# guomc9/CudaRayTracing

Measured on AMD Instinct MI355X. Metric: Mrays/sec, higher is better.
Workload: dtype f32

## Files before the change

### cudaraytracing_amd/_capi.py

```python
import ctypes as C
import os

import numpy as np

from . import build as _build

CRT_OK = 0
ERR_INVALID_ARG, ERR_NO_DEVICE, ERR_HIP = -1, -2, -3
TRAVERSAL_EXACT = 0
TRAVERSAL_REFERENCE = 1
TRAVERSAL_FAST = 2
FLAG_STATS = 1
FLAG_TILED_OUTPUT = 2
FLAG_FORCE_EXACT = 4
FLAG_TRACE_ALL = 8
FLAG_BOUNDED_RADIANCE = 16
FLAG_VARIANCE = 32
GATHER_AUTO, GATHER_RCCL, GATHER_COPY = 0, 1, 2
INTERSECT_RAW_DIRECTIONS, INTERSECT_FORCE_EXACT, INTERSECT_VISIBILITY = 0x100, 0x200, 0x400
TILE = 8


class CrtError(RuntimeError):
    def __init__(self, status, where, detail):
# ... 60 lines not shown
    def as_dict(self):
        d = {n: getattr(self, n) for n, _ in self._fields_}
        d["fallback_reason"] = d["fallback_reason"].decode("utf-8", "replace")
        return d


class BvhBuildInfo(C.Structure):
    _fields_ = [("n_triangles", C.c_uint32), ("n_nodes", C.c_uint32), ("levels", C.c_uint32), ("host_ranges", C.c_uint32),
                ("host_triangles", C.c_uint32), ("host_sorts", C.c_uint32), ("host_sort_elements", C.c_uint64), ("device_ms", C.c_float), ("total_ms", C.c_float), ("host_build_ms", C.c_float)]

    def as_dict(self):
        return {n: getattr(self, n) for n, _ in self._fields_}


class AccelInfo(C.Structure):
    _fields_ = [("n_leaves", C.c_uint32), ("n_nodes2", C.c_uint32), ("n_nodes4", C.c_uint32), ("depth2", C.c_uint32), ("depth4", C.c_uint32),
                ("sah_on_device", C.c_uint32), ("index_splits", C.c_uint32), ("sah_ms", C.c_float), ("sah_device_ms", C.c_float), ("runtime_init_ms", C.c_float), ("layout_caps", C.c_uint32)]

    def as_dict(self):
        return {n: getattr(self, n) for n, _ in self._fields_}


class TreeScalars(C.Structure):
    _fields_ = [("root_fast", C.c_int32), ("root_exact", C.c_int32), ("root3_fast", C.c_int32), ("root3_exact", C.c_int32), ("root4", C.c_int32),
                ("root4i", C.c_int32), ("n_mixed4i", C.c_uint32), ("empty4_off", C.c_uint32), ("empty4i_off", C.c_uint32), ("coord_max", C.c_float),
                ("stack_cap", C.c_uint32), ("node4i_f4", C.c_uint32)]

    def as_dict(self):
        return {n: getattr(self, n) for n, _ in self._fields_}


class AovBuffers(C.Structure):
    _fields_ = [("albedo", C.c_void_p), ("normal", C.c_void_p), ("depth", C.c_void_p), ("coverage", C.c_void_p), ("tri", C.c_void_p),
                ("material", C.c_void_p)]


class AovInfo(C.Structure):
    _fields_ = [("rays", C.c_uint64), ("chunks", C.c_uint32), ("total_ms", C.c_float)]

    def as_dict(self):
        return {n: getattr(self, n) for n, _ in self._fields_}


class DenoiseParams(C.Structure):
    _fields_ = [("width", C.c_uint32), ("height", C.c_uint32), ("iterations", C.c_uint32), ("sigma_color", C.c_float),
                ("sigma_normal", C.c_float), ("sigma_albedo", C.c_float), ("sigma_depth", C.c_float)]


class DenoiseInputs(C.Structure):
    _fields_ = [("color", C.c_void_p), ("albedo", C.c_void_p), ("normal", C.c_void_p), ("depth", C.c_void_p)]


class DenoiseVarInputs(C.Structure):
    _fields_ = [("color", C.c_void_p), ("variance", C.c_void_p), ("albedo", C.c_void_p), ("normal", C.c_void_p), ("depth", C.c_void_p)]


class DenoiseInfo(C.Structure):
    _fields_ = [("total_ms", C.c_float), ("passes", C.c_uint32)]

    def as_dict(self):
        return {n: getattr(self, n) for n, _ in self._fields_}


AOV_BUFFERS = {"albedo": (3, np.float32), "normal": (3, np.float32), "depth": (1, np.float32), "coverage": (1, np.float32),
               "tri": (1, np.int32), "material": (1, np.int32)}


class Task(C.Structure):
    _fields_ = [("n_objs", C.c_uint32), ("obj_path", (C.c_char * 512) * 8), ("mtl_dir", (C.c_char * 512) * 8),
                ("lookat", C.c_float * 3), ("up", C.c_float * 3), ("eye_pos", C.c_float * 3), ("fov_y", C.c_float),
                ("width", C.c_uint32), ("height", C.c_uint32), ("bvh_thresh_n", C.c_uint32),
                ("light_sample_n", C.c_uint32), ("spp", C.c_uint32), ("p_rr", C.c_float)]


NODE_DTYPE = np.dtype([("lc", "<i4"), ("rc", "<i4"), ("n", "<u4"), ("it", "<i4"), ("aa", "<f4", 3), ("bb", "<f4", 3)])
TRI_DTYPE = np.dtype([("v1", "<f4", 3), ("v2", "<f4", 3), ("v3", "<f4", 3), ("normal", "<f4", 3), ("area", "<f4"),
                      ("area_of_obj", "<f4"), ("material", "<i4")])
MAT_DTYPE = np.dtype([("kd", "<f4", 3), ("ke", "<f4", 3), ("ns", "<f4"), ("mode", "<i4"), ("has_emit", "<i4")])
LIGHT_DTYPE = np.dtype([("first_tri", "<u4"), ("count", "<u4")])

ABI_VERSION = 5

EXPORTS = ["crt_strerror", "crt_last_error", "crt_abi_version", "crt_device_count", "crt_scene_create",
           "crt_scene_accel_info", "crt_scene_destroy", "crt_task_obj", "crt_shard_slots", "crt_render", "crt_render_device", "crt_render_range", "crt_render_range_device", "crt_last_launch_ms", "crt_radiance_storage", "crt_preview", "crt_preview_device", "crt_variance", "crt_variance_device", "crt_render_aov", "crt_render_aov_device", "crt_denoise_defaults", "crt_denoise_scratch_bytes", "crt_denoise", "crt_denoise_device", "crt_denoise_var_defaults", "crt_denoise_var", "crt_denoise_var_device", "crt_multi_create", "crt_multi_destroy",
           "crt_multi_render", "crt_multi_frame_device", "crt_intersect",
           "crt_device_math", "crt_device_philox", "crt_device_rcp_check", "crt_scene_export", "crt_host_scene_create", "crt_host_scene_destroy",
           "crt_host_scene_add_obj", "crt_host_scene_set_bvh", "crt_host_scene_set_bvh_device", "crt_host_scene_desc", "crt_host_scene_num_objects",
           "crt_host_scene_object", "crt_inverse_view", "crt_task_load", "crt_image_load", "crt_write_png", "crt_write_pfm"]

_lib = None


def lib_path():
    return _build.LIB


def lib():
    global _lib
    if _lib is not None:
        return _lib
    path = os.environ.get("CRT_LIB_PATH") or _build.build_lib()
    L = C.CDLL(path)
    L.crt_abi_version.restype = C.c_int
    if L.crt_abi_version() != ABI_VERSION:
        raise RuntimeError("%s speaks ABI version %d, these bindings version %d (include/crt.h: CRT_ABI_VERSION)" % (path, L.crt_abi_version(), ABI_VERSION))
    L.crt_strerror.restype = C.c_char_p
    L.crt_strerror.argtypes = [C.c_int]
    L.crt_last_error.restype = C.c_char_p
    L.crt_device_count.argtypes = [C.POINTER(C.c_int)]
    L.crt_scene_create.argtypes = [C.POINTER(SceneDesc), C.c_int, C.POINTER(C.c_void_p)]
    L.crt_scene_accel_info.argtypes = [C.c_void_p, C.POINTER(AccelInfo)]
    L.crt_scene_destroy.argtypes = [C.c_void_p]
    L.crt_shard_slots.argtypes = [C.c_uint32, C.c_uint32, C.c_uint32, C.c_uint32, C.POINTER(C.c_uint64)]
    L.crt_render.argtypes = [C.c_void_p, C.POINTER(Camera), C.POINTER(Params), C.c_void_p, C.c_void_p, C.POINTER(Stats)]
    L.crt_render_device.argtypes = [C.c_void_p, C.POINTER(Camera), C.POINTER(Params), C.c_void_p, C.c_void_p,
                                    C.c_void_p, C.POINTER(Stats)]
    L.crt_render_range.argtypes = [C.c_void_p, C.POINTER(Camera), C.POINTER(Params), C.c_uint32, C.c_uint32, C.c_void_p, C.c_void_p,
                                   C.POINTER(Stats)]
    L.crt_render_range_device.argtypes = [C.c_void_p, C.POINTER(Camera), C.POINTER(Params), C.c_uint32, C.c_uint32, C.c_void_p,
                                          C.c_void_p, C.c_void_p, C.POINTER(Stats)]
    L.crt_last_launch_ms.argtypes = [C.c_void_p, C.POINTER(C.c_float), C.POINTER(C.c_uint32)]
    L.crt_radiance_storage.argtypes = [C.c_void_p, C.POINTER(C.c_uint64), C.POINTER(C.c_uint32)]
    L.crt_preview.argtypes = [C.c_void_p, C.c_void_p, C.c_void_p, C.POINTER(C.c_uint32)]
    L.crt_preview_device.argtypes = [C.c_void_p, C.c_void_p, C.c_void_p, C.c_void_p, C.POINTER(C.c_uint32)]
    L.crt_variance.argtypes = [C.c_void_p, C.c_void_p, C.POINTER(C.c_uint32)]
    L.crt_variance_device.argtypes = [C.c_void_p, C.c_void_p, C.c_void_p, C.POINTER(C.c_uint32)]
    L.crt_render_aov.argtypes = [C.c_void_p, C.POINTER(Camera), C.POINTER(Params), C.POINTER(AovBuffers), C.POINTER(AovInfo)]
    L.crt_render_aov_device.argtypes = [C.c_void_p, C.POINTER(Camera), C.POINTER(Params), C.POINTER(AovBuffers), C.c_void_p,
                                        C.POINTER(AovInfo)]
    L.crt_denoise_defaults.argtypes = [C.POINTER(DenoiseParams)]
    L.crt_denoise_scratch_bytes.argtypes = [C.c_uint32, C.c_uint32, C.POINTER(C.c_uint64)]
    L.crt_denoise.argtypes = [C.c_int, C.POINTER(DenoiseParams), C.POINTER(DenoiseInputs), C.c_void_p, C.c_void_p, C.POINTER(DenoiseInfo)]
    L.crt_denoise_device.argtypes = [C.c_int, C.POINTER(DenoiseParams), C.POINTER(DenoiseInputs), C.c_void_p, C.c_void_p, C.c_void_p, C.c_uint64,
                                     C.c_void_p, C.POINTER(DenoiseInfo)]
    L.crt_denoise_var_defaults.argtypes = [C.POINTER(DenoiseParams)]
    L.crt_denoise_var.argtypes = [C.c_int, C.POINTER(DenoiseParams), C.POINTER(DenoiseVarInputs), C.c_void_p, C.c_void_p, C.c_void_p,
                                  C.POINTER(DenoiseInfo)]
    L.crt_denoise_var_device.argtypes = [C.c_int, C.POINTER(DenoiseParams), C.POINTER(DenoiseVarInputs), C.c_void_p, C.c_void_p, C.c_void_p,
                                         C.c_void_p, C.c_uint64, C.c_void_p, C.POINTER(DenoiseInfo)]
    L.crt_multi_create.argtypes = [C.POINTER(SceneDesc), C.POINTER(C.c_int), C.c_uint32, C.c_uint32, C.POINTER(C.c_void_p)]
    L.crt_multi_destroy.argtypes = [C.c_void_p]
    L.crt_multi_render.argtypes = [C.c_void_p, C.POINTER(Camera), C.POINTER(Params), C.c_void_p, C.c_void_p, C.POINTER(Stats),
                                   C.POINTER(MultiInfo)]
    L.crt_multi_frame_device.argtypes = [C.c_void_p, C.POINTER(C.c_void_p), C.POINTER(C.c_void_p), C.POINTER(C.c_int)]
    L.crt_intersect.argtypes = [C.c_void_p, C.c_uint32, C.c_void_p, C.c_void_p, C.c_uint32, C.c_void_p, C.c_void_p]
    L.crt_device_math.argtypes = [C.c_int, C.c_char_p, C.c_uint32, C.c_void_p, C.c_void_p, C.c_void_p]
    L.crt_device_philox.argtypes = [C.c_int, C.c_uint32, C.c_void_p, C.c_void_p, C.c_void_p]
    L.crt_device_rcp_check.argtypes = [C.c_int, C.POINTER(C.c_uint64), C.POINTER(C.c_uint64)]
    L.crt_scene_export.argtypes = [C.c_void_p, C.c_char_p, C.c_void_p, C.c_size_t, C.POINTER(C.c_size_t)]
    L.crt_host_scene_create.argtypes = [C.c_uint32, C.c_uint32, C.POINTER(C.c_void_p)]
    L.crt_host_scene_destroy.argtypes = [C.c_void_p]
    L.crt_host_scene_add_obj.argtypes = [C.c_void_p, C.c_char_p, C.c_char_p]
    L.crt_host_scene_set_bvh.argtypes = [C.c_void_p, C.c_uint32]
    L.crt_host_scene_set_bvh_device.argtypes = [C.c_void_p, C.c_uint32, C.c_int, C.POINTER(BvhBuildInfo)]
    L.crt_host_scene_desc.argtypes = [C.c_void_p, C.POINTER(SceneDesc)]
    L.crt_host_scene_num_objects.argtypes = [C.c_void_p, C.POINTER(C.c_uint32)]
    L.crt_host_scene_object.argtypes = [C.c_void_p, C.c_uint32, C.POINTER(C.c_float), C.POINTER(C.c_int32),
                                        C.POINTER(C.c_uint32)]
    L.crt_inverse_view.argtypes = [C.c_void_p, C.c_void_p, C.c_void_p, C.c_void_p]
    L.crt_task_load.argtypes = [C.c_char_p, C.POINTER(Task)]
    L.crt_task_obj.argtypes = [C.c_char_p, C.c_uint32, C.c_char_p, C.c_char_p, C.c_uint32]
    L.crt_image_load.argtypes = [C.c_char_p, C.POINTER(C.c_int32), C.POINTER(C.c_int32), C.POINTER(C.c_int32), C.c_void_p, C.c_uint64]
    L.crt_write_png.argtypes = [C.c_char_p, C.c_uint32, C.c_uint32, C.c_void_p]
    L.crt_write_pfm.argtypes = [C.c_char_p, C.c_uint32, C.c_uint32, C.c_uint32, C.c_void_p]
    _lib = L
    return L


def _strerror(status):
    try:
        return lib().crt_strerror(status).decode()
    except Exception:
        return "status"


def check(status, where):
    if status != CRT_OK:
        raise CrtError(status, where, lib().crt_last_error().decode())


def ptr(a):
    return a.ctypes.data_as(C.c_void_p) if a is not None else None
```

### cudaraytracing_amd/api.py

```python
import ctypes as C
import math
import os

import numpy as np

from . import _capi as capi


def get_inverse_view_matrix(eye_pos, lookat, up):
    e = np.asarray(eye_pos, dtype=np.float32)
    l = np.asarray(lookat, dtype=np.float32)
    u = np.asarray(up, dtype=np.float32)
    out = np.zeros(9, dtype=np.float32)
    capi.check(capi.lib().crt_inverse_view(capi.ptr(e), capi.ptr(l), capi.ptr(u), capi.ptr(out)), "crt_inverse_view")
    return out


def fov_to_radians(fov_y_deg):
    return np.float32(np.float32(np.float32(fov_y_deg) * np.float32(math.pi)) / np.float32(180))


class Task:

    def __init__(self, config_path, base_dir=None):
# ... 152 lines not shown
        h = self._handle("export_trees")
        L = capi.lib()
        out = {}
        for name, dt in self.EXPORT_ARRAYS.items():
            n = C.c_size_t()
            capi.check(L.crt_scene_export(h, name.encode(), None, 0, C.byref(n)), "crt_scene_export")
            a = np.zeros(n.value // np.dtype(dt).itemsize, dtype=dt)
            if n.value:
                capi.check(L.crt_scene_export(h, name.encode(), capi.ptr(a), a.nbytes, C.byref(n)), "crt_scene_export")
            out[name] = a.reshape(-1, 4) if dt is np.float32 else a
        s = capi.TreeScalars()
        n = C.c_size_t()
        capi.check(L.crt_scene_export(h, b"scalars", C.byref(s), C.sizeof(s), C.byref(n)), "crt_scene_export")
        assert n.value == C.sizeof(s)
        out.update(s.as_dict())
        return out

    def set_spp(self, spp):
        self.spp = int(spp)

    def set_P_RR(self, p):
        self.P_RR = np.float32(p)

    def set_light_sample_n(self, n):
        self.light_sample_n = int(n)

    def _cam(self, eye_pos, inv_view_mat, fovY):
        cam = capi.Camera()
        cam.eye[:] = [float(v) for v in np.asarray(eye_pos, dtype=np.float32)]
        cam.inv_view[:] = [float(v) for v in np.asarray(inv_view_mat, dtype=np.float32).reshape(9)]
        cam.fov_y = float(np.float32(fovY))
        return cam

    def _params(self, rank=0, world=1, flags=0, width=None, height=None):
        return capi.Params(width or self.scene.width, height or self.scene.height, self.spp, float(self.P_RR),
                           self.light_sample_n, self.seed, rank, world, self.traversal, flags)

    def run_view(self, eye_pos, inv_view_mat, fovY, stats=False, want_mean=True, width=None, height=None, want_variance=False):
        if not self._h:
            raise RuntimeError("Render.run_view after free()")
        cam = self._cam(eye_pos, inv_view_mat, fovY)
        prm = self._params(flags=(capi.FLAG_STATS if stats else 0) | (capi.FLAG_VARIANCE if want_variance else 0) | self.extra_flags,
                           width=width, height=height)
        w, h = prm.width, prm.height
        rgb = np.zeros((h, w, 3), dtype=np.uint8)
        mean = np.zeros((h, w, 3), dtype=np.float32) if want_mean else None
        st = capi.Stats()
        capi.check(capi.lib().crt_render(self._h, C.byref(cam), C.byref(prm), capi.ptr(rgb), capi.ptr(mean),
                                         C.byref(st)), "crt_render")
        self.frame_buffer, self.mean_buffer, self.stats = rgb, mean, st.as_dict()
        self.variance_buffer = self.variance(width=w, height=h)[0] if want_variance else None
        return rgb

    def variance(self, width=None, height=None):
        h_ = self._handle("variance")
        w, h = width or self.scene.width, height or self.scene.height
        var = np.zeros((h, w, 3), dtype=np.float32)
        done = C.c_uint32(0)
        capi.check(capi.lib().crt_variance(h_, capi.ptr(var), C.byref(done)), "crt_variance")
        return var, int(done.value)

    def run_view_range(self, eye_pos, inv_view_mat, fovY, sample_begin, sample_count, want_mean=True, width=None, height=None,
                       want_variance=False):
        if not self._h:
            raise RuntimeError("Render.run_view_range after free()")
        cam = self._cam(eye_pos, inv_view_mat, fovY)
        prm = self._params(flags=(capi.FLAG_VARIANCE if want_variance else 0) | self.extra_flags, width=width, height=height)
        w, h = prm.width, prm.height
        last = sample_begin + sample_count == self.spp
        rgb = np.zeros((h, w, 3), dtype=np.uint8) if last else None
        mean = np.zeros((h, w, 3), dtype=np.float32) if (last and want_mean) else None
        st = capi.Stats()
        capi.check(capi.lib().crt_render_range(self._h, C.byref(cam), C.byref(prm), int(sample_begin), int(sample_count),
                                               capi.ptr(rgb) if last else None, capi.ptr(mean), C.byref(st)), "crt_render_range")
        self.stats = st.as_dict()
        if last:
            self.frame_buffer, self.mean_buffer = rgb, mean
        return rgb

    def last_launch_ms(self):
        ms, n = C.c_float(), C.c_uint32()
        capi.check(capi.lib().crt_last_launch_ms(self._handle("last_launch_ms"), C.byref(ms), C.byref(n)), "crt_last_launch_ms")
        return float(ms.value), int(n.value)

    def radiance_storage(self):
        b, r = C.c_uint64(), C.c_uint32()
        capi.check(capi.lib().crt_radiance_storage(self._handle("radiance_storage"), C.byref(b), C.byref(r)), "crt_radiance_storage")
        return int(b.value), int(r.value)

    def preview(self, want_mean=False, width=None, height=None):
        if not self._h:
            raise RuntimeError("Render.preview after free()")
        w, h = width or self.scene.width, height or self.scene.height
        rgb = np.zeros((h, w, 3), dtype=np.uint8)
        mean = np.zeros((h, w, 3), dtype=np.float32) if want_mean else None
        done = C.c_uint32(0)
        capi.check(capi.lib().crt_preview(self._h, capi.ptr(rgb), capi.ptr(mean), C.byref(done)), "crt_preview")
        return rgb, mean, int(done.value)

    def run_view_device(self, eye_pos, inv_view_mat, fovY, d_rgb_ptr, d_mean_ptr=None, stream=None, rank=0, world=1,
                        tiled=False, want_stats=True, width=None, height=None):
        self._handle("run_view_device")
        cam = self._cam(eye_pos, inv_view_mat, fovY)
        flags = (capi.FLAG_TILED_OUTPUT if (tiled or world > 1) else 0) | self.extra_flags
        prm = self._params(rank=rank, world=world, flags=flags, width=width, height=height)
        st = capi.Stats()
        capi.check(capi.lib().crt_render_device(self._h, C.byref(cam), C.byref(prm), C.c_void_p(d_rgb_ptr),
                                                C.c_void_p(d_mean_ptr) if d_mean_ptr else None,
                                                C.c_void_p(stream) if stream else None,
                                                C.byref(st) if want_stats else None), "crt_render_device")
        if want_stats:
            self.stats = st.as_dict()
        return self.stats

    def run_view_aov(self, eye_pos, inv_view_mat, fovY, want=tuple(capi.AOV_BUFFERS), width=None, height=None):
        h_ = self._handle("run_view_aov")
        cam = self._cam(eye_pos, inv_view_mat, fovY)
        prm = self._params(flags=self.extra_flags, width=width, height=height)
        w, h = prm.width, prm.height
        out, bufs = {}, capi.AovBuffers()
        for name in want:
            ch, dt = capi.AOV_BUFFERS[name]
            out[name] = np.zeros((h, w, 3) if ch == 3 else (h, w), dtype=dt)
            setattr(bufs, name, out[name].ctypes.data)
        info = capi.AovInfo()
        capi.check(capi.lib().crt_render_aov(h_, C.byref(cam), C.byref(prm), C.byref(bufs), C.byref(info)), "crt_render_aov")
        self.aov_info = info.as_dict()
        return out

    def run_view_aov_device(self, eye_pos, inv_view_mat, fovY, ptrs, stream=None, rank=0, world=1, tiled=False, want_info=True,
                            width=None, height=None):
        h_ = self._handle("run_view_aov_device")
        cam = self._cam(eye_pos, inv_view_mat, fovY)
        flags = (capi.FLAG_TILED_OUTPUT if (tiled or world > 1) else 0) | self.extra_flags
        prm = self._params(rank=rank, world=world, flags=flags, width=width, height=height)
        bufs = capi.AovBuffers()
        for name, p in ptrs.items():
            if name not in capi.AOV_BUFFERS:
                raise ValueError("unknown AOV buffer %r" % name)
            setattr(bufs, name, int(p) if p else None)
        info = capi.AovInfo()
        capi.check(capi.lib().crt_render_aov_device(h_, C.byref(cam), C.byref(prm), C.byref(bufs), C.c_void_p(stream) if stream else None,
                                                    C.byref(info) if want_info else None), "crt_render_aov_device")
        if want_info:
            self.aov_info = info.as_dict()
        return self.aov_info if want_info else None

    def run_view_denoised(self, eye_pos, inv_view_mat, fovY, iterations=None, sigma_color=None, sigma_normal=None, sigma_albedo=None,
                          sigma_depth=None, width=None, height=None, variance_guided=False):
        self._handle("run_view_denoised")
        self.run_view(eye_pos, inv_view_mat, fovY, width=width, height=height, want_variance=variance_guided)
        self.aov_buffers = self.run_view_aov(eye_pos, inv_view_mat, fovY, want=("albedo", "normal", "depth"), width=width, height=height)
        if variance_guided:
            rgb, mean, self.denoise_info = denoise_var(self.mean_buffer, self.variance_buffer, iterations=iterations, sigma_color=sigma_color,
                                                       sigma_normal=sigma_normal, sigma_albedo=sigma_albedo, sigma_depth=sigma_depth,
                                                       device=self.device, return_info=True, **self.aov_buffers)
            return rgb, mean
        rgb, mean, self.denoise_info = denoise(self.mean_buffer, iterations=iterations, sigma_color=sigma_color, sigma_normal=sigma_normal,
                                               sigma_albedo=sigma_albedo, sigma_depth=sigma_depth, device=self.device, return_info=True,
                                               **self.aov_buffers)
        return rgb, mean

    def intersect(self, origins, dirs, traversal=None):
        self._handle("intersect")
        o = np.ascontiguousarray(origins, dtype=np.float32)
        d = np.ascontiguousarray(dirs, dtype=np.float32)
# ... 293 lines not shown
```

### cudaraytracing_amd/csrc/crt_mega3.h

```cpp
#ifndef CRT_MEGA3_H
#define CRT_MEGA3_H
#include "crt_path.h"

namespace crtk {

struct MParams {
    LParams P;
    DevScene sc;
    unsigned long long* counters;
    int2* spill;
    uint32_t spill_stride;
    int32_t stack_cap;
    int32_t logic_min, leaf_min;
};

#define POOL_LV 4

#define PH3_INNER 0
#define PH3_LEAF 1
#define PH3_LA 2
#define PH3_LB 3
#define PH3_LC 4
#define PH3_N 5
#define PH3_WAIT 5
#define PH3_NONE 7
#define RF_ANYHIT 0x1000000u
#define RF_SHADOW 0x2000000u
#define RF_LAST 0x4000000u
#define RF_PROBE 0x8000000u
#define RR_ROUTE_SHIFT 25
#define RR_ROUTE_MASK 0x6000000u
#define RR_ROUTE_LC_BIT 0x4000000u
#define RF_EXACT 0x10000000u
#define RF_HASHIT 0x20000000u
#define RF_SKIP 0x40000000u
#define RF_QUERY 0x80000000u
#define POOL3_P 164
#define POOL3_QCAP ((POOL3_P + 3) & ~3)
static_assert(POOL3_P <= 256, "ray ids of a pool must fit a byte (ring entries are uint8_t)");
static_assert(POOL3_QCAP >= POOL3_P, "a ring must hold every ray of the pool");
#define CRT_MEGA3_MAX_STACK 255
#define CRT_MEGA3_MAX_LEAF 65535

typedef float v2f __attribute__((ext_vector_type(2)));

#define CRT_WAVES 4
template <bool R16_>
struct Pool3LdsT {
    static constexpr bool R16 = R16_;
    static constexpr bool DEC = false;
    static constexpr int P = POOL3_P, QCAP = POOL3_QCAP;
    static constexpr int LV = R16_ ? 2 * POOL_LV : POOL_LV;
    typedef typename std::conditional<R16_, short, int>::type stk_t;
    float4 A[POOL3_P];
    float4 B[POOL3_P];
    int node[POOL3_P];
    stk_t stk[LV][POOL3_P];
    uint32_t D[POOL3_P];
    uint8_t ring[PH3_N + 1][POOL3_QCAP];
    uint32_t waitq;
    __device__ __forceinline__ uint8_t* rq(const int p) { return ring[p]; }
};
typedef Pool3LdsT<false> Pool3Lds;
static_assert(sizeof(Pool3LdsT<true>) == sizeof(Pool3Lds), "16-bit stack entries: twice the levels in the same bytes");
static_assert(sizeof(Pool3Lds) * 4 * CRT_WAVES <= 160 * 1024, "the pool does not fit CRT_WAVES waves per SIMD into 160 KiB of LDS");

#ifndef LEAFQ_CAP
#define LEAFQ_CAP 256
#endif
static_assert((LEAFQ_CAP & (LEAFQ_CAP - 1)) == 0 && LEAFQ_CAP >= 128, "leaf queue: a power of two, room for half a batch of inner steps");
#define RD_PEND_SHIFT 8
#define RD_PEND_MASK 0x3ff00u
#define RD_FIN 0x8000000u
#define LEAF_REC_MAX 0x7fffffu
template <bool R16_, bool RING_>
struct Pool4LdsT {
    static constexpr bool R16 = R16_;
    static constexpr bool DEC = true;
    static constexpr int P = RING_ ? 148 : 152;
    static constexpr int QCAP = (P + 3) & ~3;
    static constexpr int LV = R16_ ? 6 : 3;
    typedef typename std::conditional<R16_, short, int>::type stk_t;
    float4 A[P];
    float4 B[P];
    unsigned long long best[P];
    stk_t stk[LV][P];
    uint32_t D[P];
    uint32_t leafq[LEAFQ_CAP + 1];
    uint8_t ring[(RING_ ? 5 : 4)][QCAP];
    uint32_t waitq;
    __device__ __forceinline__ uint8_t* rq(const int p) { return ring[p == PH3_INNER ? 0 : p - 1]; }
};
static_assert(sizeof(Pool4LdsT<true, false>) * 4 * CRT_WAVES <= 160 * 1024 && sizeof(Pool4LdsT<true, true>) * 4 * CRT_WAVES <= 160 * 1024 &&
              sizeof(Pool4LdsT<false, false>) * 4 * CRT_WAVES <= 160 * 1024 && sizeof(Pool4LdsT<false, true>) * 4 * CRT_WAVES <= 160 * 1024,
              "the DEC pool does not fit CRT_WAVES waves per SIMD into 160 KiB of LDS");
static_assert(Pool4LdsT<true, false>::P <= 256, "ray ids of a pool must fit a byte");

struct MParams3 {
    MParams M;
    int* spill;
    uint32_t force_exact;
    int32_t dbg_loads, dbg_valu;
};

static_assert(offsetof(MParams3, dbg_loads) == 748 && offsetof(MParams3, dbg_valu) == 752, "tools/bbprof/instrument.py reads the counter buffer's address from these two kernel-argument dwords");


typedef void (*Mega3Kernel)(const MParams3);
Mega3Kernel mega3_kernel(int mode, bool stats, bool all, bool query, bool r16, bool ring = false, bool dec = false, bool impl = false);
uint32_t mega3_pool_p(bool dec, bool ring);
int mega3_lds_levels(bool dec, bool r16);
bool bbprof_launch(Mega3Kernel kern, MParams3 M3, uint32_t blocks, hipStream_t st);
void launch_order_items(bool ring, uint32_t blocks, hipStream_t st, const LParams& P, uint32_t* list, unsigned int* cnt);

}
#endif
```

### cudaraytracing_amd/csrc/crt_mega3.hip

```cpp
#include "crt_internal.h"

#include <cstdio>
#include <cstdlib>
#include <cstring>
#include <vector>

namespace crtk {

struct NewRay {
    F3 o, d;
    float tl;
    uint32_t kind, flags;
};

__device__ __forceinline__ float fmin3(float a, float b, float c) { return __builtin_fminf(__builtin_fminf(a, b), c); }
__device__ __forceinline__ float fmax3(float a, float b, float c) { return __builtin_fmaxf(__builtin_fmaxf(a, b), c); }
__device__ __forceinline__ v2f v2(float a, float b) { v2f r; r.x = a; r.y = b; return r; }
__device__ __forceinline__ v2f v2s(float a) { v2f r; r.x = a; r.y = a; return r; }

__device__ __forceinline__ int smax(const int a, const int b)
{
    int r;
    asm("s_max_i32 %0, %1, %2" : "=s"(r) : "s"(a), "s"(b) : "scc");
    return r;
// ... 39 lines not shown
    uint32_t flags = (nr.flags & ~(RF_SKIP | RF_SHADOW | RF_LAST | RF_PROBE)) | route_bits(nr.flags);
    const float max_o = __builtin_elementwise_maximum(__builtin_elementwise_maximum(absf(nr.o.x), absf(nr.o.y)), absf(nr.o.z));
    const float max_inv = __builtin_elementwise_maximum(__builtin_elementwise_maximum(absf(inv.x), absf(inv.y)), absf(inv.z));
    const bool finite = ((sc.coord_max + max_o) * max_inv <= 0x1p126f) & finite3(nr.d.x, nr.d.y, nr.d.z);
    if (MODE == 1 || !finite || force_exact) flags |= RF_EXACT;
    const int ref = (MODE != 1 && finite && !force_exact) ? (IMPL ? sc.root4i : sc.root4) : sc.root3_exact;
    bool answered = false;
    float T = FLT_MAX;
    if (MODE != 1 && nr.kind == RAY_SHADOW) {
        flags |= RF_ANYHIT;
        T = nr.tl;
        answered = !(nr.tl == nr.tl) || nr.tl == -pinf() || (nr.flags & RF_SKIP) != 0;
    }
    if constexpr (LDS::DEC) {
        static_assert(!LDS::DEC || MODE == 2, "decoupled leaves: CRT_TRAVERSAL_EXACT");
        if (ref < 0) flags |= RF_EXACT;
        S.A[id] = make_float4(nr.o.x, nr.o.y, nr.o.z, (flags & RF_ANYHIT) ? T : pinf());
        S.B[id] = make_float4(nr.d.x, nr.d.y, nr.d.z, __int_as_float(ref));
        S.best[id] = (unsigned long long)0x7f7fffffu << 32;
        S.D[id] = flags;
        enters_exact = false;
        if (answered) return route_done<QUERY>(flags);
        enters_exact = (flags & RF_EXACT) != 0;
        return PH3_INNER;
    } else {
    S.A[id] = make_float4(nr.o.x, nr.o.y, nr.o.z, T);
    S.B[id] = make_float4(nr.d.x, nr.d.y, nr.d.z, __int_as_float(-1));
    S.node[id] = ref;
    S.D[id] = flags;
    enters_exact = false;
    if (answered) return route_done<QUERY>(flags);
    enters_exact = MODE != 1 && (flags & RF_EXACT) != 0;
    return ref >= 0 ? PH3_INNER : PH3_LEAF;
    }
}

template <class LDS>
__device__ __forceinline__ void ray_result(LDS& S, const uint32_t id, float4& qa, float4& qb)
{
    qa = S.A[id]; qb = S.B[id];
    if constexpr (LDS::DEC) {
        const unsigned long long b = S.best[id];
        qa.w = __uint_as_float((uint32_t)(b >> 32));
        qb.w = __uint_as_float(~(uint32_t)b);
    }
}
template <bool QUERY>
__device__ __forceinline__ uint32_t route_complete(const uint32_t rec_flags, const bool has_hit)
{
    if (QUERY) return PH3_LC;
    const uint32_t r = (rec_flags >> RR_ROUTE_SHIFT) & 3u;
    return (has_hit ? (r & 1u) : r) + (uint32_t)PH3_LA;
}

template <int MODE>
__device__ __forceinline__ bool shadow_blocked(float tl, float T, int tri)
{
    if (MODE != 1) return tri >= 0 || tl - FLT_MAX > CRT_EPSILON;
    return tl - T > CRT_EPSILON;
}

__device__ __forceinline__ F3 finish_path_m3(const LParams& P, const Tables<false>& tb, const uint32_t slot, const int deepest, const bool emissive, const F3 ke,
                                            const bool have_ld, const F3 ld)
{
    const Pool& pl = P.pool;
    F3 L = f3(0.0f, 0.0f, 0.0f);
    if (deepest < 0) return L;
    const float inv_pdf_sphere = (float)(2.0f * 3.14159265358979323846);
    if (emissive) {
        L = deepest == 0 ? add3(f3(0.0f, 0.0f, 0.0f), ke) : f3(0.0f, 0.0f, 0.0f);
    } else if (have_ld) {
        L = add3(f3(0.0f, 0.0f, 0.0f), ld);
    } else {
        const float4 a = gld_rec(&pl.rec_a[(size_t)deepest * pl.n + slot]);
        L = add3(f3(0.0f, 0.0f, 0.0f), f3(a.x, a.y, a.z));
    }
    for (int v = deepest - 1; v >= 0; v -= CRT_FINISH_PF) {
        float4 a[CRT_FINISH_PF], fm[CRT_FINISH_PF];
        float cs[CRT_FINISH_PF];
#pragma unroll
        for (int j = 0; j < CRT_FINISH_PF; j++) {
            const int vj = v - j > 0 ? v - j : 0;
            a[j] = gld_rec(&pl.rec_a[(size_t)vj * pl.n + slot]);
            cs[j] = __uint_as_float(gld((const uint32_t*)&pl.rec_b[(size_t)vj * pl.n + slot].w));
        }
#pragma unroll
        for (int j = 0; j < CRT_FINISH_PF; j++) fm[j] = mat_row(tb, TNM_MAT(__float_as_uint(a[j].w)), 0);
#pragma unroll
        for (int j = 0; j < CRT_FINISH_PF; j++) {
            if (v - j >= 0) {
                F3 ind = mul3(L, f3(fm[j].x, fm[j].y, fm[j].z));
                ind = scale3(ind, cs[j]);
                ind = scale3(ind, inv_pdf_sphere);
                ind = div3(ind, P.p_rr);
                L = add3(ind, f3(a[j].x, a[j].y, a[j].z));
            }
        }
    }
    return L;
}

__device__ __forceinline__ bool shadow_blocked_bit(const bool tl_inf, const int tri) { return tri >= 0 || tl_inf; }
#define ST_TL_INF (1u << 12)

template <int MODE, bool RING = false>
__device__ __forceinline__ uint32_t logic_A(const LParams& P, const Tables<false>& tb, const uint32_t g, const float4 qa, const float4 qb, NewRay& nr,
                                            PathCounters& cnt, const bool trace_all)
{
    const DevScene& sc = P.sc;
    const Pool& pl = P.pool;
    constexpr bool TRI_CC = MODE != 1;
    const float4 la = gld(&pl.la[g]);
    const uint4 idv = load_path_id<RING, !TRI_CC>(P, g);
    const float4 cc = gld(&pl.cc[g]);
    const uint32_t st = __float_as_uint(la.w);
    const uint32_t stage = (st >> 8) & 15u;
    const uint32_t vtri_old = TRI_CC ? ((st & 0xfffu) == ((uint32_t)ST_HIT << 8) ? 0u : __float_as_uint(cc.w)) : idv.w;
    const float4 vn = gld(&sc.tri_nm[vtri_old]);
    const float res_t = qa.w;
    const int res_tri = __float_as_int(qb.w);
    const float4 gq_hit = gld(&sc.tri_nm[res_tri >= 0 ? res_tri : 0]);
    const uint32_t mat_old = min(TNM_MAT(__float_as_uint(vn.w)), P.n_mats - 1u);
    const uint32_t mat_cur = stage == ST_HIT ? TNM_MAT(__float_as_uint(gq_hit.w)) : mat_old;
    uint32_t tnm_cur = stage == ST_HIT ? __float_as_uint(gq_hit.w) : __float_as_uint(vn.w);
    float4 m0_cur = mat_row(tb, mat_cur, 0);
    const uint32_t n_nee = (uint32_t)(sc.n_lights * P.lsn);
    const uint32_t q_next = stage == ST_SHADOW ? (st >> 16) + 1 : 0u;
    uint4 lg_next = make_uint4(0u, 1u, 0u, 0u);
    if (n_nee > 0) {
        if (sc.n_lights == 1) {
            const crt_u4v_ l0_ = *(const __attribute__((address_space(4))) crt_u4v_*)tb.lights;
            lg_next = make_uint4(l0_.x, l0_.y, l0_.z, l0_.w);
        } else lg_next = gld(&tb.lights[fast_div(q_next < n_nee ? q_next : 0u, P.lsn_div.m, P.lsn_div.sh)]);
    }
    Lane s;
    s.depth = st & 255u; s.q = st >> 16; s.stage = stage;
    s.Ld = f3(la.x, la.y, la.z);
    s.nrm = f3(vn.x, vn.y, vn.z); s.mat = TNM_MAT(__float_as_uint(vn.w));
    s.pixel_index = idv.x; s.k = idv.y; s.item = idv.z;
    s.ro = f3(qa.x, qa.y, qa.z); s.tl = 0.0f;
    s.rd = f3(qb.x, qb.y, qb.z);
    s.pos = s.ro; s.vtri = vtri_old; s.c = f3(0.0f, 0.0f, 0.0f); s.kind = RAY_NONE;
    bool do_enter = false;
    if (stage == ST_SHADOW) {
        const bool blocked = TRI_CC ? shadow_blocked_bit((st & ST_TL_INF) != 0u, res_tri) : shadow_blocked<MODE>(cc.w, res_t, res_tri);
        if (!blocked) s.Ld = add3(s.Ld, f3(cc.x, cc.y, cc.z));
        s.q++;
    } else if (stage == ST_HIT) {
        const F3 pos = add3(s.ro, scalel3(res_t, s.rd));
        do_enter = true;
        if (s.depth > 0) {
            const size_t pr = (size_t)(s.depth - 1) * pl.n + g;
            const F3 pn = s.nrm;
            float cos_prev = dot3(unit3(sub3(pos, s.ro)), pn);
            cos_prev = cos_prev > 0.0f ? cos_prev : 0.0f;
            gst_rec(&pl.rec_b[pr].w, cos_prev);
            if (TNM_SPECULAR(__float_as_uint(vn.w))) {
                const float ns = mat_row(tb, s.mat, 0).w;
                const float4 pb = gld_rec(&pl.rec_b[pr]);
                const float delta_coeff = (float)((double)(det_expf(25 / ns) - 1) / (2.71828182845904523536 - 1));
                const F3 in = unit3(f3(pb.x, pb.y, pb.z));
                const F3 out = sub3(in, scale3(pn, 2.f * dot3(in, pn)));
                const float d_theta = (float)((double)(delta_coeff * 30) * 3.14159265358979323846 / 180);
                const float d_phi = (float)((double)(delta_coeff * 120) * 3.14159265358979323846 / 180);
                const U4 rp = rng_draw(P.seed, s.pixel_index, s.k, s.depth - 1, RNG_PROBE, 0);
                const F3 refd = unit3(sample_lobe(out, d_theta, d_phi, rng_uniform(rp.x), rng_uniform(rp.y)));
                gst_rec(&pl.rec_b[(size_t)s.depth * pl.n + g], make_float4(s.rd.x, s.rd.y, s.rd.z, 0.0f));
                gst(&pl.vx[g], make_float4(pos.x, pos.y, pos.z, __int_as_float(res_tri)));
                gst(&pl.la[g], make_float4(s.Ld.x, s.Ld.y, s.Ld.z, __uint_as_float(s.depth | ((uint32_t)ST_PROBE << 8) | (s.q << 16))));
                nr.o = s.ro; nr.d = unit3(refd);  nr.tl = 0.0f; nr.kind = RAY_CLOSEST; nr.flags = RF_PROBE;
                return PH3_NONE;
            }
        }
        s.pos = pos; s.vtri = (uint32_t)res_tri;
    } else {
        const float4 vx = gld(&pl.vx[g]);
        s.pos = f3(vx.x, vx.y, vx.z); s.vtri = __float_as_uint(vx.w);
        if (res_tri >= 0) {
            const int hmat = gld(&sc.tri_mat[res_tri]);
            const float4 h1 = mat_row(tb, hmat, 1);
            if (__float_as_uint(h1.w) & 1u) {
                const float4 h2 = mat_row(tb, hmat, 2);
                const size_t pr = (size_t)(s.depth - 1) * pl.n + g;
                const F3 pn = s.nrm;
                const float4 pm0 = mat_row(tb, s.mat, 0), pm1 = mat_row(tb, s.mat, 1);
                const float log_shininess = det_log10f(pm0.w);
                const float shininess_coeff = (float)((double)log_shininess * 0.5 + 1);
                const float ip = (float)(2.0f * 3.14159265358979323846) / 8.f;
                const F3 hp = add3(s.ro, scalel3(res_t, s.rd));
                float ct = dot3(unit3(sub3(hp, s.ro)), pn);
                ct = ct > 0.0f ? ct : 0.0f;
                const F3 kekd = mul3(f3(h2.x, h2.y, h2.z), f3(pm1.x, pm1.y, pm1.z));
                const F3 temp = scale3(scale3(scalel3(shininess_coeff, kekd), ct), ip);
                float4 a = gld_rec(&pl.rec_a[pr]);
                a.x = a.x + temp.x; a.y = a.y + temp.y; a.z = a.z + temp.z;
                gst_rec(&pl.rec_a[pr], a);
            }
        }
        const float4 pb = gld_rec(&pl.rec_b[(size_t)s.depth * pl.n + g]);
        s.rd = f3(pb.x, pb.y, pb.z);
        do_enter = true;
    }
    if (do_enter) {
        float4 gq = gq_hit;
        if (stage == ST_PROBE) {
            gq = gld(&sc.tri_nm[s.vtri]);
            m0_cur = mat_row(tb, TNM_MAT(__float_as_uint(gq.w)), 0); tnm_cur = __float_as_uint(gq.w);
        }
        s.nrm = f3(gq.x, gq.y, gq.z);
        s.mat = TNM_MAT(__float_as_uint(gq.w));
        if (TNM_SPECULAR(tnm_cur)) gst_rec(&pl.rec_b[(size_t)s.depth * pl.n + g], make_float4(s.rd.x, s.rd.y, s.rd.z, 0.0f));
        if (!TRI_CC) store_path_tri(P, g, s.vtri);
        if (TNM_EMITTER(tnm_cur)) {
            gst(&pl.la[g], make_float4(TRI_CC ? __uint_as_float(s.vtri) : 0.0f, 0.0f, 0.0f, __uint_as_float(s.depth | ((uint32_t)ST_FIN << 8) | (1u << 16))));
            return PH3_LC;
        }
        s.Ld = f3(0.0f, 0.0f, 0.0f);
        s.q = 0;
        if (n_nee == 0) {
            gst(&pl.la[g], make_float4(0.0f, 0.0f, 0.0f, __uint_as_float(s.depth | ((uint32_t)ST_NEED << 8))));
            if (TRI_CC) gst(&pl.cc[g].w, __uint_as_float(s.vtri));
            nr.o = s.pos;
            return PH3_LB;
        }
    }
    constexpr int LA_LOOP_MIN = 16;
    const float4 m0 = m0_cur;
    bool skip;
    for (bool first = true;; first = false) {
        if (first) setup_shadow_lg(P, s, f3(m0.x, m0.y, m0.z), lg_next);
        else setup_shadow(P, tb, s, f3(m0.x, m0.y, m0.z));
        skip = MODE != 1 && !trace_all && (s.c.x == 0.0f && s.c.y == 0.0f && s.c.z == 0.0f);
        if (!skip) break;
        cnt.untraced++;
        if (__popcll(__builtin_amdgcn_ballot_w64(true)) < LA_LOOP_MIN) break;
        cnt.rays++; cnt.shadow++;
        s.q++;
        if (s.q == n_nee) {
            gst(&pl.la[g], make_float4(s.Ld.x, s.Ld.y, s.Ld.z, __uint_as_float(s.depth | ((uint32_t)ST_NEED << 8))));
            if (TRI_CC) gst(&pl.cc[g].w, __uint_as_float(s.vtri));
            nr.o = s.pos;
            return PH3_LB;
        }
    }
    gst(&pl.la[g], make_float4(s.Ld.x, s.Ld.y, s.Ld.z, __uint_as_float(s.depth | ((uint32_t)ST_SHADOW << 8) | (s.q << 16) | ((TRI_CC && s.tl == pinf()) ? ST_TL_INF : 0u))));
    gst(&pl.cc[g], make_float4(s.c.x, s.c.y, s.c.z, TRI_CC ? __uint_as_float(s.vtri) : s.tl));
    nr.o = s.ro; nr.d = s.rd; nr.tl = s.tl; nr.kind = RAY_SHADOW;
    nr.flags = RF_SHADOW | (s.q + 1 == n_nee ? RF_LAST : 0u) | (skip ? RF_SKIP : 0u);
    return PH3_NONE;
}

template <int MODE, bool RING = false>
__device__ __forceinline__ uint32_t logic_B(const LParams& P, const uint32_t g, const float4 qa, const float4 qb, NewRay& nr)
{
    const Pool& pl = P.pool;
    constexpr bool TRI_CC = MODE != 1;
    const float4 la = gld(&pl.la[g]);
    const uint4 idv = load_path_id<RING, !TRI_CC>(P, g);
    const float4 cc = gld(&pl.cc[g]);
    const uint32_t st = __float_as_uint(la.w);
    const uint32_t stage = (st >> 8) & 15u;
    uint32_t depth = st & 255u;
    F3 Ld = f3(la.x, la.y, la.z);
    if (stage == ST_SHADOW) {
        const bool blocked = TRI_CC ? shadow_blocked_bit((st & ST_TL_INF) != 0u, __float_as_int(qb.w)) : shadow_blocked<MODE>(cc.w, qa.w, __float_as_int(qb.w));
        if (!blocked) Ld = add3(Ld, f3(cc.x, cc.y, cc.z));
    }
    bool stop = depth == CRT_BOUNCE_STACK_SIZE - 1;
    U4 rb;
    rb.x = rb.y = rb.z = rb.w = 0;
    if (!stop) {
        rb = rng_draw(P.seed, idv.x, idv.y, depth, RNG_BOUNCE, 0);
        stop = rng_uniform(rb.x) > P.p_rr;
    }
    if (stop) {
        gst(&pl.la[g], make_float4(Ld.x, Ld.y, Ld.z, __uint_as_float(depth | ((uint32_t)ST_FIN << 8))));
        return PH3_LC;
    }
    const float4 vn = gld(&P.sc.tri_nm[TRI_CC ? __float_as_uint(cc.w) : idv.w]);
    const float4 vx = qa;
    gst_rec(&pl.rec_a[(size_t)depth * pl.n + g], make_float4(Ld.x, Ld.y, Ld.z, vn.w));
    const F3 ndir = unit3(sample_hemisphere(f3(vn.x, vn.y, vn.z), rng_uniform(rb.y), rng_uniform(rb.z)));
    depth++;
    gst(&pl.la[g], make_float4(Ld.x, Ld.y, Ld.z, __uint_as_float(depth | ((uint32_t)ST_HIT << 8))));
    nr.o = f3(vx.x, vx.y, vx.z); nr.d = unit3(ndir);  nr.tl = 0.0f; nr.kind = RAY_CLOSEST; nr.flags = 0;
    return PH3_NONE;
}

enum { LC_DEAD = 0, LC_RAY = 1, LC_WAIT = 2 };
template <int MODE, bool RING>
__device__ __forceinline__ int logic_C(const LParams& P, const Tables<false>& tb, const uint32_t g, PathCounters& cnt, NewRay& nr, uint32_t& fin_key)
{
    constexpr bool TRI_CC = MODE != 1;
    const Pool& pl = P.pool;
    const float4 la = gld(&pl.la[g]);
    const uint4 idv = load_path_id<RING, !TRI_CC>(P, g);
    const uint32_t st = __float_as_uint(la.w);
    const uint32_t stage = (st >> 8) & 15u;
    const uint32_t depth = st & 255u;
    constexpr bool ring = RING;
    const bool waiting = ring && stage == ST_WAIT;
    const uint32_t home_ = RING ? blockIdx.x & (P.ring_shards - 1u) : blockIdx.x & (ITEM_SHARDS - 1);
    const uint32_t lo_ = home_ * P.items_per_shard, hi_ = min(lo_ + P.items_per_shard, P.n_items);
    const unsigned long long gmask_ = __ballot(!waiting);
    const int lane_ = threadIdx.x & 63;
    const uint32_t grank_ = (uint32_t)__popcll(gmask_ & ((1ull << lane_) - 1ull));
    unsigned int pre_base_ = 0;
    const bool pre_ok_ = lo_ < P.n_items && gmask_ != 0ull;
    if (pre_ok_ && lane_ == __ffsll((long long)gmask_) - 1) pre_base_ = __hip_atomic_fetch_add((CRT_GAS unsigned int*)(P.item_next + home_ * ITEM_STRIDE), (unsigned int)__popcll(gmask_), __ATOMIC_RELAXED, __HIP_MEMORY_SCOPE_AGENT);
    uint32_t home_word_ = 0;
    if (RING) home_word_ = ring_load(P.ring_state + home_ * ITEM_STRIDE);
    if (stage != ST_NEW && !waiting) {
        int deepest = (int)depth;
        bool emissive = false;
        F3 ke = f3(0.0f, 0.0f, 0.0f);
        if (stage == ST_HIT) deepest = (int)depth - 1;
        else if ((st >> 16) & 1u) {
            emissive = true;
            const float4 m2 = mat_row(tb, TNM_MAT(__float_as_uint(gld(&P.sc.tri_nm[TRI_CC ? __float_as_uint(la.x) : idv.w]).w)), 2);
            ke = f3(m2.x, m2.y, m2.z);
        }
        const F3 L = finish_path_m3(P, tb, g, deepest, emissive, ke, stage == ST_FIN && !emissive, f3(la.x, la.y, la.z));
        if (ring) {
            const uint32_t sh = fast_div(idv.z, P.items_per_shard_div.m, P.items_per_shard_div.sh), c = idv.z - sh * P.items_per_shard;
            const uint32_t s = fast_div(c, P.spsh_div.m, P.spsh_div.sh), rs = s & P.ring_mask;
            float4* Lr = P.L + (size_t)rs * P.ring_stride + (size_t)sh * P.spsh + (c - s * P.spsh);
            ring_store16(Lr, L.x, L.y, L.z);
            fin_key = (sh << 16) | rs;
        } else {
            typedef float f4v_ __attribute__((ext_vector_type(4)));
            f4v_ Lv_; Lv_.x = L.x; Lv_.y = L.y; Lv_.z = L.z; Lv_.w = 0.0f;
            __builtin_nontemporal_store(Lv_, (CRT_GAS f4v_*)&P.L[idv.z]);
        }
    }
    bool first_ = pre_ok_ && !waiting;
    for (;;) {
        uint32_t item = ITEM_NONE;
        if (waiting) item = idv.z;
        else {
            if (first_) {
                const unsigned long long idx_ = (unsigned long long)lo_ + (unsigned int)__builtin_amdgcn_readfirstlane((int)pre_base_) + grank_;
                if (idx_ < hi_) item = (uint32_t)idx_;
                first_ = false;
            }
            if (item == ITEM_NONE) item = RING ? grab_item_ring(P.item_next, P.items_per_shard, P.ring_shards, home_)
                                               : grab_item(nullptr, P.item_next, P.items_per_shard, P.n_items, blockIdx.x & (ITEM_SHARDS - 1));
            if (item == ITEM_NONE) return LC_DEAD;
            if (P.item_list) {
                const uint32_t sh_ = fast_div(item, P.items_per_shard_div.m, P.items_per_shard_div.sh);
                const uint32_t slo_ = sh_ * P.items_per_shard, shi_ = min(slo_ + P.items_per_shard, P.n_items);
                const uint32_t wlo_ = shi_ - min(P.order_window, shi_ - slo_);
                if (item >= wlo_) item = __hip_atomic_load((CRT_GAS const unsigned int*)&P.item_list[sh_ * P.order_window + (item - wlo_)], __ATOMIC_RELAXED, __HIP_MEMORY_SCOPE_AGENT);
            }
        }
        bool valid; uint32_t pi, pj, pixel_index, k;
        decode_item<RING>(P, item, pixel_index, k, valid, pi, pj);
        if (!valid) continue;
        if (ring && !ring_gate_open(P, item, home_, home_word_)) {
            if (!waiting) {
                store_path_id<!TRI_CC>(P, g, item);
                gst(&pl.la[g], make_float4(0.0f, 0.0f, 0.0f, __uint_as_float((uint32_t)ST_WAIT << 8)));
            }
            return LC_WAIT;
        }
        cnt.paths++;
        if (!waiting) store_path_id<!TRI_CC>(P, g, item);
        const F3 wd = camera_dir(P, pixel_index, k, pi, pj);
        gst(&pl.la[g], make_float4(0.0f, 0.0f, 0.0f, __uint_as_float((uint32_t)ST_HIT << 8)));
        nr.o = f3(P.eye[0], P.eye[1], P.eye[2]); nr.d = unit3(wd);  nr.tl = 0.0f; nr.kind = RAY_CLOSEST; nr.flags = 0;
        return LC_RAY;
    }
}

__device__ __forceinline__ bool query_C(const LParams& P, const uint32_t g, const float4 qa, const float4 qb, NewRay& nr)
{
    const Pool& pl = P.pool;
    const float4 la = gld(&pl.la[g]);
    const uint4 idv = load_path_id(P, g);
    if (((__float_as_uint(la.w) >> 8) & 15u) != ST_NEW) gst(&P.L[idv.z], make_float4(qa.w, qb.w, 0.0f, 0.0f));
    const uint32_t item = grab_item(nullptr, P.item_next, P.items_per_shard, P.n_items, blockIdx.x & (ITEM_SHARDS - 1));
    if (item == ITEM_NONE) return false;
    store_path_id(P, g, item);
    gst(&pl.la[g], make_float4(0.0f, 0.0f, 0.0f, __uint_as_float((uint32_t)ST_HIT << 8)));
    const float4 o = gld(&P.q_o[item]), d = gld(&P.q_d[item]);
    nr.o = f3(o.x, o.y, o.z); nr.d = f3(d.x, d.y, d.z); nr.tl = o.w; nr.kind = __float_as_uint(d.w); nr.flags = RF_QUERY;
    return true;
}

__device__ __forceinline__ void slab_pair(const float4 n0, const float4 n1, const float4 n2, const F3 o, const F3 inv, const F3 d, const bool exact,
                                          bool& hl, bool& hr, float& tl, float& tr)
{
    const v2f tx0 = (v2(n0.x, n0.y) - v2s(o.x)) * v2s(inv.x), ty0 = (v2(n0.z, n0.w) - v2s(o.y)) * v2s(inv.y), tz0 = (v2(n1.x, n1.y) - v2s(o.z)) * v2s(inv.z);
    const v2f tx1 = (v2(n1.z, n1.w) - v2s(o.x)) * v2s(inv.x), ty1 = (v2(n2.x, n2.y) - v2s(o.y)) * v2s(inv.y), tz1 = (v2(n2.z, n2.w) - v2s(o.z)) * v2s(inv.z);
    float el, er, xl, xr;
    if (!exact) {
        el = fmax3(__builtin_fminf(tx0.x, tx1.x), __builtin_fminf(ty0.x, ty1.x), __builtin_fminf(tz0.x, tz1.x));
        er = fmax3(__builtin_fminf(tx0.y, tx1.y), __builtin_fminf(ty0.y, ty1.y), __builtin_fminf(tz0.y, tz1.y));
        xl = fmin3(__builtin_fmaxf(tx0.x, tx1.x), __builtin_fmaxf(ty0.x, ty1.x), __builtin_fmaxf(tz0.x, tz1.x));
        xr = fmin3(__builtin_fmaxf(tx0.y, tx1.y), __builtin_fmaxf(ty0.y, ty1.y), __builtin_fmaxf(tz0.y, tz1.y));
    } else {
        const bool nx = d.x < 0, ny = d.y < 0, nz = d.z < 0;
        el = maxf_ref(maxf_ref(nx ? tx1.x : tx0.x, ny ? ty1.x : ty0.x), nz ? tz1.x : tz0.x);
        er = maxf_ref(maxf_ref(nx ? tx1.y : tx0.y, ny ? ty1.y : ty0.y), nz ? tz1.y : tz0.y);
        xl = minf_ref(minf_ref(nx ? tx0.x : tx1.x, ny ? ty0.x : ty1.x), nz ? tz0.x : tz1.x);
        xr = minf_ref(minf_ref(nx ? tx0.y : tx1.y, ny ? ty0.y : ty1.y), nz ? tz0.y : tz1.y);
    }
    hl = (el <= xl + CRT_EPSILON) & (xl >= 0);
    hr = (er <= xr + CRT_EPSILON) & (xr >= 0);
    tl = el; tr = er;
}

__device__ __forceinline__ void slab_pair_pruned(const float4 n0, const float4 n1, const float4 n2, const F3 o, const F3 inv, const float bound,
                                                 float& tl, float& tr)
{
    const v2f tx0 = (v2(n0.x, n0.y) - v2s(o.x)) * v2s(inv.x), ty0 = (v2(n0.z, n0.w) - v2s(o.y)) * v2s(inv.y), tz0 = (v2(n1.x, n1.y) - v2s(o.z)) * v2s(inv.z);
    const v2f tx1 = (v2(n1.z, n1.w) - v2s(o.x)) * v2s(inv.x), ty1 = (v2(n2.x, n2.y) - v2s(o.y)) * v2s(inv.y), tz1 = (v2(n2.z, n2.w) - v2s(o.z)) * v2s(inv.z);
    const float el = fmax3(__builtin_fminf(tx0.x, tx1.x), __builtin_fminf(ty0.x, ty1.x), __builtin_fminf(tz0.x, tz1.x));
    const float er = fmax3(__builtin_fminf(tx0.y, tx1.y), __builtin_fminf(ty0.y, ty1.y), __builtin_fminf(tz0.y, tz1.y));
    const float xl = fmin3(__builtin_fmaxf(tx0.x, tx1.x), __builtin_fmaxf(ty0.x, ty1.x), __builtin_fmaxf(tz0.x, tz1.x));
    const float xr = fmin3(__builtin_fmaxf(tx0.y, tx1.y), __builtin_fmaxf(ty0.y, ty1.y), __builtin_fmaxf(tz0.y, tz1.y));
    const float inf = pinf();
    tl = ((el <= __builtin_fminf(xl + CRT_EPSILON, bound)) & (xl >= 0)) ? el : inf;
    tr = ((er <= __builtin_fminf(xr + CRT_EPSILON, bound)) & (xr >= 0)) ? er : inf;
}

template <bool PRUNE = true>
__device__ __forceinline__ void slab_quad_pruned(const float4 nx, const float4 fx, const float4 ny, const float4 fy, const float4 nz, const float4 fz,
                                                 const F3 o, const F3 inv, const float bound, float& t0, float& t1, float& t2, float& t3)
{
    const v2f nxa = (v2(nx.x, nx.y) - v2s(o.x)) * v2s(inv.x), nxb = (v2(nx.z, nx.w) - v2s(o.x)) * v2s(inv.x);
    const v2f nya = (v2(ny.x, ny.y) - v2s(o.y)) * v2s(inv.y), nyb = (v2(ny.z, ny.w) - v2s(o.y)) * v2s(inv.y);
    const v2f nza = (v2(nz.x, nz.y) - v2s(o.z)) * v2s(inv.z), nzb = (v2(nz.z, nz.w) - v2s(o.z)) * v2s(inv.z);
    const v2f fxa = (v2(fx.x, fx.y) - v2s(o.x)) * v2s(inv.x), fxb = (v2(fx.z, fx.w) - v2s(o.x)) * v2s(inv.x);
    const v2f fya = (v2(fy.x, fy.y) - v2s(o.y)) * v2s(inv.y), fyb = (v2(fy.z, fy.w) - v2s(o.y)) * v2s(inv.y);
    const v2f fza = (v2(fz.x, fz.y) - v2s(o.z)) * v2s(inv.z), fzb = (v2(fz.z, fz.w) - v2s(o.z)) * v2s(inv.z);
    const float e0 = fmax3(nxa.x, nya.x, nza.x), e1 = fmax3(nxa.y, nya.y, nza.y), e2 = fmax3(nxb.x, nyb.x, nzb.x), e3 = fmax3(nxb.y, nyb.y, nzb.y);
    const float x0 = fmin3(fxa.x, fya.x, fza.x), x1 = fmin3(fxa.y, fya.y, fza.y), x2 = fmin3(fxb.x, fyb.x, fzb.x), x3 = fmin3(fxb.y, fyb.y, fzb.y);
    const float inf = pinf();
    if (PRUNE) {
        t0 = ((e0 <= __builtin_fminf(x0 + CRT_EPSILON, bound)) & (x0 >= 0)) ? e0 : inf;
        t1 = ((e1 <= __builtin_fminf(x1 + CRT_EPSILON, bound)) & (x1 >= 0)) ? e1 : inf;
        t2 = ((e2 <= __builtin_fminf(x2 + CRT_EPSILON, bound)) & (x2 >= 0)) ? e2 : inf;
        t3 = ((e3 <= __builtin_fminf(x3 + CRT_EPSILON, bound)) & (x3 >= 0)) ? e3 : inf;
    } else {
        t0 = ((e0 <= x0 + CRT_EPSILON) & (x0 >= 0)) ? e0 : inf;
        t1 = ((e1 <= x1 + CRT_EPSILON) & (x1 >= 0)) ? e1 : inf;
        t2 = ((e2 <= x2 + CRT_EPSILON) & (x2 >= 0)) ? e2 : inf;
        t3 = ((e3 <= x3 + CRT_EPSILON) & (x3 >= 0)) ? e3 : inf;
    }
}

// ... 316 lines not shown
}

template <int MODE, bool STATS, class LDS>
__device__ __forceinline__ bool inner2_step(const DevScene& sc, LDS& S, const MParams3& M, const uint32_t id, const uint32_t g, const F3 o, const F3 inv,
                                            const F3 d, const float bound, int& ref, int& sp, TravCounters& tc, uint32_t& max_sp)
{
    const float4* nd = sc.nodes3 + (size_t)ref * 4;
    const float4 n0 = nd[0], n1 = nd[1], n2 = nd[2];
    const float2 n3 = *(const float2*)(nd + 3);
    if (STATS) tc.inner++;
    bool hl, hr;
    float tl, tr;
    slab_pair(n0, n1, n2, o, inv, d, true, hl, hr, tl, tr);
    const int lref = __float_as_int(n3.x), rref = __float_as_int(n3.y);
    bool left_first;
    if (MODE == 1) {
        left_first = false;
    } else {
        hl = hl && !(tl > bound);
        hr = hr && !(tr > bound);
        left_first = tl <= tr;
    }
    const bool both = hl && hr, any = hl || hr;
    const int near_ref = both ? (left_first ? lref : rref) : (hl ? lref : rref);
    const int lv = lds_levels<LDS>(true);
    if (both) {
        stack_push(S, M, id, g, sp, left_first ? rref : lref, lv);
        if (STATS && (uint32_t)sp > max_sp) max_sp = (uint32_t)sp;
    }
    if (any) { ref = near_ref; return false; }
    return stack_pop(S, M, id, g, sp, ref, lv);
}

#define CRT_SORT4(mode) ((mode) != 2)
template <int MODE, bool STATS, bool ALL = false, bool QUERY = false, bool R16 = false, bool RING = false, bool DEC = false, bool IMPL = false>
__global__ __launch_bounds__(64) __attribute__((amdgpu_waves_per_eu(CRT_WAVES, CRT_WAVES))) void k_mega3(const MParams3 M3)
{
    static_assert(!IMPL || (DEC && R16), "the tree without its rows of refs: decoupled leaves, 16-bit stack entries");
    static_assert(!(RING && (QUERY || STATS)), "the commit ring is a render without counters");
    static_assert(!(R16 && MODE == 1), "CRT_TRAVERSAL_REFERENCE walks the 2-wide trees: 32-bit stack entries");
    static_assert(!DEC || MODE == 2, "decoupled leaves: CRT_TRAVERSAL_EXACT");
    typedef typename std::conditional<DEC, Pool4LdsT<R16, RING>, Pool3LdsT<R16>>::type LDS3;
    __shared__ LDS3 S;
    constexpr int QCAP = LDS3::QCAP;
    const MParams& M = M3.M;
    const LParams& P = M.P;
    const DevScene& sc = P.sc;
    const Pool& pl = P.pool;
    const int lane = threadIdx.x;
    const uint32_t base = blockIdx.x * (uint32_t)LDS3::P;
    Tables<false> tb;
    tb.mats = sc.mats; tb.lights = sc.lights;

    PathCounters cnt;
    cnt = PathCounters{};
    TravCounters tc;
    tc.inner = tc.leaf = tc.tests = tc.hits = 0;
    uint32_t max_sp = 0;
    int n_exact = 0;

    int qn[PH3_N];
#pragma unroll
    for (int p = 0; p < PH3_N; p++) qn[p] = 0;
    uint32_t dg_b[5] = {0, 0, 0, 0, 0}, dg_l[5] = {0, 0, 0, 0, 0};
    uint32_t dg_sp[6] = {0, 0, 0, 0, 0, 0};
    uint32_t dg_ov[2] = {0, 0};
    uint32_t lq_h = 0, lq_t = 0;
    constexpr bool commit_ring = RING;
#ifdef CRT_STAMPS
    unsigned long long st_acc[6] = {0, 0, 0, 0, 0, 0};
    uint32_t st_n[6] = {0, 0, 0, 0, 0, 0};
    unsigned long long st_prev = __builtin_amdgcn_s_memtime();
#define STAMP(k_) { const unsigned long long t_ = __builtin_amdgcn_s_memtime(); st_acc[k_] += t_ - st_prev; st_prev = t_; st_n[k_]++; }
#define STAMP_OTHER() { const unsigned long long t_ = __builtin_amdgcn_s_memtime(); st_acc[3] += t_ - st_prev; st_prev = t_; }
#else
#define STAMP(k_)
#define STAMP_OTHER()
#endif
    if (commit_ring && lane == 0) S.waitq = 0u;
    {
        const int n_valid = __builtin_amdgcn_readfirstlane((int)min((uint32_t)LDS3::P, pl.n > base ? pl.n - base : 0u));
        for (int i = lane; i < n_valid; i += 64) {
            S.rq(PH3_LC)[i] = (uint8_t)i;
            pl.la[base + i] = make_float4(0.0f, 0.0f, 0.0f, __uint_as_float((uint32_t)ST_NEW << 8));
        }
        qn[PH3_LC] = n_valid;
    }

#define PUSH3()                                                                                                            \
    _Pragma("unroll") for (int p = 0; p < PH3_N; p++) {                                                                    \
        const bool mine = nph == (uint32_t)p;                                                                         \
        const unsigned long long m = __ballot(mine);                                                                       \
        if (m) {                                                                                                           \
                  \
            const uint32_t slot = __builtin_amdgcn_mbcnt_hi((uint32_t)(m >> 32), __builtin_amdgcn_mbcnt_lo((uint32_t)m, RQ_PUSH_BASE(p))); \
            if (mine) S.rq(p)[slot] = (uint8_t)id;                                                                             \
            const int add = (int)__popcll(m);                                                                              \
            RQ_PUSH_ADV(p, add)                                                                                            \
        }                                                                                                                  \
    }
#define PUSH_TRAV() { if (on) nph = t_done ? route_done<QUERY>(t_flags) : (t_ref >= 0 ? PH3_INNER : PH3_LEAF); PUSH3() }
#define POP3(p)                                                                                                            \
    const int take = min(64, qn[p]);                                                                                       \
    if (STATS) { dg_b[p]++; dg_l[p] += (uint32_t)take; }                                                                   \
    const bool on = lane < take;                                                                                           \
    const uint32_t id = S.rq(p)[RQ_POP_BASE(p, take) + (uint32_t)lane];                                                        \
    RQ_POP_ADV(p, take)                                                                                                    \
    const uint32_t g = base + id;                                                                                          \
    uint32_t nph = PH3_NONE;

#define LOGIC_PARAMS()                                                                                                     \
    const __attribute__((address_space(4))) char* ka_ = (const __attribute__((address_space(4))) char*)__builtin_amdgcn_kernarg_segment_ptr(); \
    asm volatile("" : "+s"(ka_));                                                                                          \
    union { LParams p; uint32_t w[sizeof(LParams) / 4]; } pu_;                                                             \
    {                                                                                                                      \
        const __attribute__((address_space(4))) uint32_t* src_ =                                                           \
            (const __attribute__((address_space(4))) uint32_t*)(ka_ + offsetof(MParams3, M) + offsetof(MParams, P));       \
        _Pragma("unroll") for (unsigned i_ = 0; i_ < sizeof(LParams) / 4; i_++) pu_.w[i_] = src_[i_];                      \
    }                                                                                                                      \
    const LParams& Pl = pu_.p;                                                                                             \
    Tables<false> tl;                                                                                                      \
    tl.mats = Pl.sc.mats; tl.lights = Pl.sc.lights;

    for (;;) {
      int act;
      for (;;) {
        {
            const int kC = min(qn[PH3_LC], 64) * 8 + PH3_LC, kA = min(qn[PH3_LA], 64) * 8 + PH3_LA, kB = min(qn[PH3_LB], 64) * 8 + PH3_LB;
#define LEAFQ_FIRST 48
            static_assert(LEAFQ_FIRST >= 1 && LEAFQ_FIRST + 64 + 4 <= LEAFQ_CAP, "leaf queue: LEAFQ_FIRST - 1 entries + a reference-arithmetic batch + one lane's four entries must fit LEAFQ_CAP");
            const int nl_ = DEC ? (int)(lq_t - lq_h) : qn[PH3_LEAF];
            const int kL = ((DEC && nl_ >= LEAFQ_FIRST) ? 64 : min(nl_, 64)) * 8 + PH3_LEAF, kI = min(qn[PH3_INNER], 64) * 8 + PH3_INNER;
            const int best = STATS ? max(max(max(kC, kA), max(kB, kL)), kI)
                                   : smax(smax(smax(kC, kA), smax(kB, kL)), kI);
            act = best < 8 ? PH3_NONE : (best & 7);
        }
        if (act > PH3_LEAF) break;
        auto inner_arm = [&](auto may_exact_) __attribute__((always_inline)) {
            constexpr bool MAY_EXACT = decltype(may_exact_)::value;
            if constexpr (!DEC) {
            POP3(PH3_INNER)
            bool t_done = false;
            int t_ref = 0;
            uint32_t t_flags = 0;
            if (on) {
                const float4 qa = S.A[id], qbd = S.B[id];
                const uint32_t qd = S.D[id];
                int ref = S.node[id];
                constexpr bool DIR_ = MODE == 2 && !MAY_EXACT;
                const F3 o = f3(qa.x, qa.y, qa.z), inv = DIR_ ? f3(qbd.x, qbd.y, qbd.z) : inv3_exact(f3(qbd.x, qbd.y, qbd.z));
                int sp = (int)(qd & 0xffu);
                const float bound = (MODE == 0 && (qd & (RF_ANYHIT | RF_HASHIT))) ? prune_bound(qa.w, o, inv) : pinf();
                bool done = false;
                if (MODE == 1) {
                    const float4 qb = S.B[id];
                    done = inner2_step<1, STATS>(sc, S, M3, id, g, o, inv, f3(qb.x, qb.y, qb.z), bound, ref, sp, tc, max_sp);
                } else if (!MAY_EXACT) {
                    done = inner4_step<STATS, CRT_SORT4(MODE), LDS3, DIR_>(sc, S, M3, id, g, o, inv, bound, ref, sp, tc, max_sp);
                } else {
                    const bool ex = (qd & RF_EXACT) != 0;
                    if (!ex) done = inner4_step<STATS, CRT_SORT4(MODE)>(sc, S, M3, id, g, o, inv, bound, ref, sp, tc, max_sp);
                    if (__builtin_amdgcn_ballot_w64(ex)) {
                        if (ex) {
                            const float4 qb = S.B[id];
                            done = inner2_step<0, STATS>(sc, S, M3, id, g, o, inv, f3(qb.x, qb.y, qb.z), bound, ref, sp, tc, max_sp);
                        }
                    }
// ... 560 lines not shown
```

### cudaraytracing_amd/csrc/crt_path.h

```cpp
#ifndef CRT_PATH_H
#define CRT_PATH_H
#include "../../include/crt.h"
#include "crt_accel.h"
#include "crt_device.h"
#include "crt_trace.h"

#include <hip/hip_runtime.h>

#include <cfloat>
#include <cstddef>
#include <cstdint>
#include <type_traits>

namespace crtk {
using namespace crtdev;

enum { C_RAYS = 0, C_SHADOW, C_PROBE, C_INNER, C_LEAF, C_TESTS, C_HITS, C_PATHS, C_ALIVE, C_MAXSP, C_SUMSP, C_CYC_LOGIC, C_CYC_LEAF, C_CYC_INNER, C_CYC_OTHER,
       C_DIAG , C_UNTRACED = C_DIAG + 20, C_COUNT };
#define CNT_SHARDS 256
#define CNT_STRIDE 40
#define ITEM_SHARDS 64
#define ITEM_STRIDE 32

enum { ST_DEAD = 0, ST_NEW = 1, ST_HIT = 2, ST_PROBE = 3, ST_SHADOW = 4, ST_FIN = 5, ST_NEED = 6, ST_WAIT = 7, ST_COUNT_ };
static_assert(ST_COUNT_ <= 16, "a stage is kept in 4 bits");
enum { RAY_NONE = 0, RAY_CLOSEST = 1, RAY_SHADOW = 2 };
#define ITEM_NONE 0xffffffffu

struct Pool {
    float4* ro;
    float4* rd;
    float4* vx;
    float4* la;
    float4* cc;
    float4* vn;
    uint4* id;
    float2* res;
    float4* rec_a;
    float4* rec_b;
    uint32_t n;
};

struct LParams {
    DevScene sc;
    Pool pool;
    float eye[3];
    float inv_view[9];
    float scale, ar;
    uint32_t width, height;
    float p_rr;
    int32_t lsn;
    float inv_lsn_pow2;
    uint32_t pad_;
    uint64_t seed;
    uint32_t rank, world, tiles_x, n_tiles;
    uint32_t nslots;
    uint32_t sample_begin;
    uint32_t n_items;
    uint32_t items_per_shard;
    uint32_t n_mats;
    FastDiv lsn_div, nslots_div, tiles_x_div;
    unsigned int* item_next;
    float4* L;
    unsigned long long* counters;
    const float4* q_o;
    const float4* q_d;
    const uint32_t* item_list;
    uint32_t order_window;
    FastDiv items_per_shard_div;
    uint32_t ring_mask;
    uint32_t spsh;
    FastDiv spsh_div;
    uint32_t ring_shards;
    uint32_t ring_stride;
    uint32_t n_samples;
    uint32_t tail_first;
    float spp_f;
    uint32_t ring_pad_;
    unsigned int* ring_done;
    unsigned int* ring_state;
    float* accum;
};

struct TParams {
    DevScene sc;
    Pool pool;
    unsigned long long* counters;
    unsigned int* slot_next;
    uint32_t slots_per_shard;
    int32_t stack_cap;
    int2* spill;
    uint32_t spill_stride;
    int32_t refill_min, leaf_min;
};

__device__ __forceinline__ bool slot_to_pixel(uint32_t slot, uint32_t rank, uint32_t world, uint32_t n_tiles, uint32_t tiles_x, FastDiv tiles_x_div,
                                              uint32_t width, uint32_t height, uint32_t& i, uint32_t& j)
{
    uint32_t tile = (slot >> 6) * world + rank;
    uint32_t pix = slot & 63u;
    if (tile >= n_tiles) return false;
    uint32_t ty = fast_div(tile, tiles_x_div.m, tiles_x_div.sh), tx = tile - ty * tiles_x;
    i = tx * CRT_TILE + (pix & 7u);
    j = ty * CRT_TILE + (pix >> 3);
    return i < width && j < height;
}

#define CRT_GAS __attribute__((address_space(1)))
typedef float crt_f4v_ __attribute__((ext_vector_type(4)));
typedef uint32_t crt_u4v_ __attribute__((ext_vector_type(4)));
__device__ __forceinline__ float4 gld(const float4* p) { const crt_f4v_ v = *(const CRT_GAS crt_f4v_*)p; return make_float4(v.x, v.y, v.z, v.w); }
__device__ __forceinline__ uint4 gld(const uint4* p) { const crt_u4v_ v = *(const CRT_GAS crt_u4v_*)p; return make_uint4(v.x, v.y, v.z, v.w); }
__device__ __forceinline__ int32_t gld(const int32_t* p) { return *(const CRT_GAS int32_t*)p; }
__device__ __forceinline__ uint32_t gld(const uint32_t* p) { return *(const CRT_GAS uint32_t*)p; }
__device__ __forceinline__ void gst(float4* p, const float4 v) { crt_f4v_ t; t.x = v.x; t.y = v.y; t.z = v.z; t.w = v.w; *(CRT_GAS crt_f4v_*)p = t; }
__device__ __forceinline__ void gst(uint4* p, const uint4 v) { crt_u4v_ t; t.x = v.x; t.y = v.y; t.z = v.z; t.w = v.w; *(CRT_GAS crt_u4v_*)p = t; }
__device__ __forceinline__ void gst(float* p, const float v) { *(CRT_GAS float*)p = v; }
__device__ __forceinline__ float4 gld_rec(const float4* p) { return gld(p); }
__device__ __forceinline__ void gst_rec(float4* p, const float4 v) { gst(p, v); }
__device__ __forceinline__ void gst_rec(float* p, const float v) { gst(p, v); }

__device__ __forceinline__ uint32_t grab_item(const unsigned int* , unsigned int* item_next, uint32_t per, uint32_t n_items,
                                              uint32_t home)
{
    const int lane = threadIdx.x & 63;
    uint32_t item = ITEM_NONE;
    for (uint32_t t = 0; t < ITEM_SHARDS; t++) {
        const uint32_t sh = (home + t) & (ITEM_SHARDS - 1);
        const uint32_t lo = sh * per;
        if (lo >= n_items) continue;
        const uint32_t hi = min(lo + per, n_items);
        unsigned int* cur = item_next + sh * ITEM_STRIDE;
        if (lo + __hip_atomic_load((CRT_GAS unsigned int*)cur, __ATOMIC_RELAXED, __HIP_MEMORY_SCOPE_AGENT) >= hi) continue;
        const unsigned long long mask = __ballot(1);
        const int leader = __ffsll((long long)mask) - 1;
        const uint32_t rank = (uint32_t)__popcll(mask & ((1ull << lane) - 1ull));
// ... 339 lines not shown
```

### cudaraytracing_amd/csrc/crt_render.hip

```cpp
#include "crt_internal.h"

#include <algorithm>
#include <cfloat>
#include <chrono>
#include <cstdio>
#include <cstdlib>
#include <cstring>
#include <limits>
#include <string>
#include <type_traits>
#include <array>
#include <atomic>
#include <vector>

using namespace crtdev;
using namespace crtk;

struct crt_scene {
    int device = 0;
    DevBuf<float4> nodes, tri_geo, mats, ltri, nodes3, leaf_geo, tri_nm, nodes4, nodes4i, leaf_geo_i;
    DevBuf<int32_t> rec_map;
    bool impl_ok = false;
    int depth4 = 1;
    bool ref16_ok = false;
    bool ref16_inner_ok = false;
    bool dec_ok = false;
    uint32_t max_leaf = 0;
    DevBuf<int32_t> tri_mat, leaf_count;
    DevBuf<uint4> lights;
    DevBuf<float4> p_ro, p_rd, p_vx, p_la, p_cc, p_vn, p_rec_a, p_rec_b, L;
    DevBuf<uint4> p_id;
    uint32_t n_mats = 0;
    DevBuf<float2> p_res;
    DevBuf<float> accum;
    DevBuf<float4> aov_acc;
    DevBuf<unsigned long long> counters;
    DevBuf<unsigned int> item_next;
    DevBuf<uint32_t> item_list;
    DevBuf<unsigned int> ring_done, ring_state;
    DevBuf<float4> ring_L;
    std::vector<unsigned int> ring_state_host;
    uint64_t last_radiance_bytes = 0;
    uint32_t last_ring_samples = 0;
    DevBuf<unsigned int> order_cnt;
    DevBuf<unsigned int> slot_next[2];
    DevBuf<int2> spill[2];
    hipStream_t aux_stream = nullptr;
    hipEvent_t ev_fork = nullptr, ev_join = nullptr;
    hipEvent_t ev_k0 = nullptr, ev_k1 = nullptr;
    uint32_t last_launches = 0;
    int n_cus = 0;
    unsigned long long* h_counters = nullptr;
    DevScene dev{};
    int stack_cap = 0;
    uint32_t n_tris = 0;
    crt_accel_info accel{};
    struct { uint32_t samples = 0, spp = 0, width = 0, height = 0, rank = 0, world = 1, tiled = 0; } acc;
    DevBuf<float> accum_q;
    struct { uint32_t samples = 0, spp = 0, width = 0, height = 0, rank = 0, world = 1, tiled = 0; bool valid = false; } var;
    std::vector<hipEvent_t> ev;
    ~crt_scene()
    {
        for (hipEvent_t e : ev) (void)hipEventDestroy(e);
        if (ev_k0) (void)hipEventDestroy(ev_k0);
        if (ev_k1) (void)hipEventDestroy(ev_k1);
        if (ev_fork) (void)hipEventDestroy(ev_fork);
        if (ev_join) (void)hipEventDestroy(ev_join);
        if (aux_stream) (void)hipStreamDestroy(aux_stream);
        if (h_counters) (void)hipHostFree(h_counters);
    }
};

static bool use_ref16(const crt_scene* sc, int mode, bool dec = false)
{
    if (mode == 1 || !(dec ? sc->ref16_inner_ok : sc->ref16_ok)) return false;
    const char* e = std::getenv("CRT_REF16");
    const char* f = std::getenv("CRT_REF32");
    if (f && f[0] == '1') return false;
    return dec || !(e && e[0] == '0');
}

namespace {

int fail(int status, const std::string& msg)
{
    crt_set_last_error_(msg.c_str());
    return status;
}
int fail_hip(const HipFail& f)
{
    return fail(CRT_ERR_HIP, std::string(f.what) + ": " + hipGetErrorString(f.e));
}

float as_float(int32_t v) { float f; std::memcpy(&f, &v, 4); return f; }
int32_t as_int(float f) { int32_t v; std::memcpy(&v, &f, 4); return v; }

struct AccelInfo {
    uint32_t n_leaves = 0, n_nodes2 = 0, on_device = 0, index_splits = 0;
    float sah_ms = 0.0f, sah_device_ms = 0.0f;
};
int convert_bvh(const crt_scene_desc& d, std::vector<float4>& nodes, std::vector<int32_t>& leaf_count, int32_t& root_fast, int32_t& root_exact, AccelInfo* ai = nullptr)
{
    auto is_leaf = [&](int32_t i) { return d.nodes[i].lc < 0 && d.nodes[i].rc < 0; };
    auto leaf_ref = [&](int32_t i) -> int32_t {
        const crt_bvh_node& n = d.nodes[i];
        uint32_t cnt = n.n <= 15 ? n.n : 0;
        if (n.n > 15) leaf_count[n.it] = (int32_t)n.n;
        return (int32_t)~(((uint32_t)n.it << 4) | cnt);
    };
    leaf_count.assign(d.n_tris ? d.n_tris : 1, 0);
    nodes.clear();
    if (is_leaf(d.root)) { root_fast = root_exact = leaf_ref(d.root); return 1; }

    std::vector<crtaccel::Prim> prims;
    for (uint32_t i = 0; i < d.n_nodes; i++) {
        if (!is_leaf((int32_t)i)) continue;
        crtaccel::Prim p;
        for (int a = 0; a < 3; a++) { p.box.lo[a] = d.nodes[i].aa[a]; p.box.hi[a] = d.nodes[i].bb[a]; }
        p.ref = leaf_ref((int32_t)i);
        prims.push_back(p);
    }
    std::vector<crtaccel::Node> acc;
    int32_t acc_root = 0;
    const auto sah_t0 = std::chrono::steady_clock::now();
    int depth_fast = -1;
// ... 63 lines not shown
int validate_desc(const crt_scene_desc* d)
{
    if (!d || !d->nodes || !d->tris || !d->materials || d->n_nodes == 0 || d->n_tris == 0 || d->n_materials == 0)
        return fail(CRT_ERR_INVALID_ARG, "crt_scene_create: empty scene description");
    if (d->root < 0 || (uint32_t)d->root >= d->n_nodes) return fail(CRT_ERR_INVALID_ARG, "crt_scene_create: root index out of range");
    if (d->n_tris >= (1u << 27)) return fail(CRT_ERR_UNSUPPORTED, "crt_scene_create: more than 2^27 triangles");
    if (d->n_lights && (!d->lights || !d->light_tris)) return fail(CRT_ERR_INVALID_ARG, "crt_scene_create: lights without triangles");
    for (uint32_t i = 0; i < d->n_nodes; i++) {
        const crt_bvh_node& n = d->nodes[i];
        bool leaf = n.lc < 0 && n.rc < 0;
        if (leaf) {
            if (n.it < 0 || n.n == 0 || (uint64_t)n.it + n.n > d->n_tris) return fail(CRT_ERR_INVALID_ARG, "crt_scene_create: leaf range outside the triangle array");
        } else {
            if (n.lc < 0 || n.rc < 0 || (uint32_t)n.lc >= i || (uint32_t)n.rc >= i) return fail(CRT_ERR_INVALID_ARG, "crt_scene_create: inner node children must precede it (post-order)");
        }
    }
    {
        std::vector<uint8_t> seen(d->n_nodes, 0), owned(d->n_tris, 0);
        std::vector<int32_t> todo(1, d->root);
        uint32_t visited = 0;
        while (!todo.empty()) {
            const int32_t i = todo.back();
            todo.pop_back();
            if (seen[i]) return fail(CRT_ERR_INVALID_ARG, "crt_scene_create: a node is reachable from the root more than once");
            seen[i] = 1;
            visited++;
            const crt_bvh_node& n = d->nodes[i];
            if (n.lc < 0 && n.rc < 0) {
                for (uint32_t k = 0; k < n.n; k++) {
                    if (owned[(uint32_t)n.it + k]) return fail(CRT_ERR_INVALID_ARG, "crt_scene_create: two leaves share a triangle");
                    owned[(uint32_t)n.it + k] = 1;
                }
            } else { todo.push_back(n.lc); todo.push_back(n.rc); }
        }
        if (visited != d->n_nodes) return fail(CRT_ERR_INVALID_ARG, "crt_scene_create: nodes that the root does not reach");
    }
    if (d->n_materials >= (1u << 30)) return fail(CRT_ERR_INVALID_ARG, "crt_scene_create: more than 2^30 - 1 materials (the triangle rows keep two flag bits beside the index)");
    for (uint32_t i = 0; i < d->n_tris; i++)
        if (d->tris[i].material < 0 || (uint32_t)d->tris[i].material >= d->n_materials) return fail(CRT_ERR_INVALID_ARG, "crt_scene_create: triangle material index out of range");
    for (uint32_t i = 0; i < d->n_light_tris; i++)
        if (d->light_tris[i].material < 0 || (uint32_t)d->light_tris[i].material >= d->n_materials) return fail(CRT_ERR_INVALID_ARG, "crt_scene_create: light triangle material index out of range");
    for (uint32_t i = 0; i < d->n_lights; i++)
        if (d->lights[i].count == 0 || (uint64_t)d->lights[i].first_tri + d->lights[i].count > d->n_light_tris) return fail(CRT_ERR_INVALID_ARG, "crt_scene_create: light range outside the light triangle array");
    return CRT_OK;
}

struct Shard {
    uint32_t tiles_x, tiles_y, n_tiles, local_tiles, nslots;
};
struct RingPlan { uint32_t samples, spsh, shards; };
Shard make_shard(uint32_t w, uint32_t h, uint32_t world)
{
    Shard s;
    s.tiles_x = (w + CRT_TILE - 1) / CRT_TILE;
    s.tiles_y = (h + CRT_TILE - 1) / CRT_TILE;
    s.n_tiles = s.tiles_x * s.tiles_y;
    s.local_tiles = (s.n_tiles + world - 1) / world;
    s.nslots = s.local_tiles * 64u;
    return s;
}

float inv_if_pow2(int32_t n) { return (n > 0 && (n & (n - 1)) == 0) ? 1.0f / (float)n : 0.0f; }

uint32_t env_u32(const char* name, uint32_t dflt)
{
    const char* v = std::getenv(name);
    if (!v || !*v) return dflt;
    long x = std::strtol(v, nullptr, 10);
    return x > 0 ? (uint32_t)x : dflt;
}

static bool use_dec(const crt_scene* sc, int mode)
{
    if (mode != 2 || !sc->dec_ok) return false;
    const char* e = std::getenv("CRT_DEC");
    if (e && e[0] == '0') return false;
    return true;
}
static bool use_impl(const crt_scene* sc, bool dec, bool r16)
{
    if (!dec || !r16 || !sc->impl_ok) return false;
    const char* e = std::getenv("CRT_IMPL");
    return !(e && e[0] == '0');
}
uint32_t choose_pipeline(const crt_scene* sc);

void camera_scale_ar(const crt_camera* cam, const crt_params* prm, float& scale, float& ar)
{
    scale = det_tanf(cam->fov_y / 2);
    ar = (float)prm->width / (float)prm->height;
}

const uint64_t kMaxChunkItems = 1ull << 30;

struct TraceSetup {
    TParams T;
    size_t lds;
    int mode_id;
    uint32_t blocks;
};
TraceSetup make_trace_setup(crt_scene* sc, const Pool& pool, uint32_t traversal, bool want_stats, int half = 0, int n_halves = 1)
{
    TraceSetup S;
    std::memset(&S.T, 0, sizeof(S.T));
    TParams& T = S.T;
    T.sc = sc->dev; T.pool = pool; T.counters = sc->counters.p;
    T.slot_next = sc->slot_next[half].p;
    T.refill_min = (int32_t)std::min<uint32_t>(64, env_u32("CRT_REFILL_MIN", REFILL_MIN));
    T.leaf_min = (int32_t)std::min<uint32_t>(64, env_u32("CRT_LEAF_MIN", LEAF_MIN));
    T.slots_per_shard = ((pool.n + SLOT_SHARDS - 1) / SLOT_SHARDS + 63u) & ~63u;
    const int lds_cap = (int)std::min<uint32_t>((uint32_t)sc->stack_cap, std::max(2u, env_u32("CRT_STACK_LDS", 8)));
    T.stack_cap = lds_cap;
    S.lds = (size_t)lds_cap * 256 * sizeof(int2);
    S.mode_id = (traversal == CRT_TRAVERSAL_REFERENCE ? 2 : traversal == CRT_TRAVERSAL_EXACT ? 4 : 0) + (want_stats ? 1 : 0);
    int per_cu = trace_blocks_per_cu(S.mode_id, S.lds);
    const uint32_t dflt_per_cu = n_halves > 1 ? 3u : 64u;
    per_cu = (int)std::min<uint32_t>((uint32_t)per_cu, env_u32("CRT_TRACE_BLOCKS_PER_CU", dflt_per_cu));
    S.blocks = std::min<uint32_t>((pool.n + 255) / 256, (uint32_t)(sc->n_cus * per_cu));
    const int spill_levels = std::max(1, sc->stack_cap - lds_cap);
    T.spill_stride = S.blocks * 256u;
    sc->spill[half].ensure((size_t)spill_levels * T.spill_stride);
    T.spill = sc->spill[half].p;
    return S;
}
void launch_trace_pass(crt_scene* sc, const TraceSetup& S, hipStream_t st)
{
    HIP_CHECK(hipMemsetAsync(S.T.slot_next, 0, (size_t)SLOT_SHARDS * SLOT_STRIDE * sizeof(unsigned int), st));
    launch_trace(S.mode_id, S.T, S.blocks, S.lds, st);
}

const float* trace_queries(crt_scene* sc, uint32_t n, uint32_t traversal, bool force_exact, hipStream_t st, uint32_t& stride)
{
    if (choose_pipeline(sc) == 4) {
        const bool reference = traversal == CRT_TRAVERSAL_REFERENCE;
        int per_cu = 1;
        const bool exact = traversal == CRT_TRAVERSAL_EXACT;
        const int mode3 = reference ? 1 : exact ? 2 : 0;
        const bool dec = use_dec(sc, mode3);
        const bool r16 = use_ref16(sc, mode3, dec);
        const Mega3Kernel kern3 = mega3_kernel(mode3, false, false, true, r16, false, dec, use_impl(sc, dec, r16));
        if (hipOccupancyMaxActiveBlocksPerMultiprocessor(&per_cu, kern3, 64, 0) != hipSuccess || per_cu < 1) per_cu = 1;
        const uint32_t pool_p = mega3_pool_p(dec, false);
        const uint32_t blocks = std::min<uint32_t>((n + pool_p - 1) / pool_p, (uint32_t)(sc->n_cus * per_cu));
        const uint32_t lanes = blocks * pool_p;
        sc->p_la.ensure(lanes); sc->p_id.ensure(lanes); sc->L.ensure(n);
        sc->spill[0].ensure((size_t)(r16 ? std::max(1, sc->stack_cap) : std::max(1, sc->stack_cap - mega3_lds_levels(dec, r16))) * lanes);
        MParams3 M3;
        std::memset(&M3, 0, sizeof(M3));
        LParams& P = M3.M.P;
        P.sc = sc->dev;
        P.pool.la = sc->p_la.p; P.pool.id = sc->p_id.p; P.pool.n = lanes;
        P.n_items = n;
        P.items_per_shard = ((n + ITEM_SHARDS - 1) / ITEM_SHARDS + 63u) & ~63u;
        P.item_next = sc->item_next.p; P.L = sc->L.p; P.counters = sc->counters.p;
        P.q_o = sc->p_ro.p; P.q_d = sc->p_rd.p;
        P.nslots = 1; P.nslots_div = make_fastdiv(1); P.tiles_x = 1; P.tiles_x_div = make_fastdiv(1); P.lsn_div = make_fastdiv(1);
        M3.M.sc = sc->dev; M3.M.counters = sc->counters.p; M3.M.spill_stride = lanes; M3.M.stack_cap = mega3_lds_levels(dec, r16);
        M3.spill = (int*)sc->spill[0].p;
        M3.force_exact = force_exact ? 1u : 0u;
        HIP_CHECK(hipMemsetAsync(sc->item_next.p, 0, (size_t)ITEM_SHARDS * ITEM_STRIDE * sizeof(unsigned int), st));
        hipLaunchKernelGGL(kern3, dim3(blocks), dim3(64), 0, st, M3);
        HIP_CHECK(hipGetLastError());
        stride = 4;
        return (const float*)sc->L.p;
    }
    Pool pool;
    std::memset(&pool, 0, sizeof(pool));
    pool.ro = sc->p_ro.p; pool.rd = sc->p_rd.p; pool.res = sc->p_res.p; pool.n = n;
    TraceSetup TS = make_trace_setup(sc, pool, traversal, false);
    launch_trace_pass(sc, TS, st);
    HIP_CHECK(hipGetLastError());
    stride = 2;
    return (const float*)sc->p_res.p;
}

int render_impl(crt_scene* sc, const crt_camera* cam, const crt_params* prm, void* d_rgb, void* d_mean, hipStream_t st, crt_stats* stats,
                uint32_t s_begin = 0, uint32_t s_count = 0xffffffffu)
{
    if (!sc || !cam || !prm) return fail(CRT_ERR_INVALID_ARG, "crt_render: null argument");
    if (s_count == 0xffffffffu) s_count = prm->spp > s_begin ? prm->spp - s_begin : 0;
    if (s_count == 0 || (uint64_t)s_begin + s_count > prm->spp) return fail(CRT_ERR_INVALID_ARG, "crt_render: sample range outside [0, spp)");
    const uint32_t s_end = s_begin + s_count;
    if (!d_rgb && s_end == prm->spp) return fail(CRT_ERR_INVALID_ARG, "crt_render: null frame buffer");
    if (prm->width == 0 || prm->height == 0 || prm->spp == 0) return fail(CRT_ERR_INVALID_ARG, "crt_render: width, height and spp must be positive");
    if (prm->world == 0 || prm->rank >= prm->world) return fail(CRT_ERR_INVALID_ARG, "crt_render: need rank < world");
    if (prm->light_sample_n < 0 || prm->light_sample_n > 4096) return fail(CRT_ERR_INVALID_ARG, "crt_render: light_sample_n must be in [0, 4096]");
    if ((uint64_t)prm->width * prm->height > 0xffffffffull) return fail(CRT_ERR_UNSUPPORTED, "crt_render: more than 2^32 pixels");
    if (prm->traversal != CRT_TRAVERSAL_FAST && prm->traversal != CRT_TRAVERSAL_REFERENCE && prm->traversal != CRT_TRAVERSAL_EXACT)
        return fail(CRT_ERR_INVALID_ARG, "crt_render: unknown traversal mode");
    const bool want_stats = (prm->flags & CRT_FLAG_STATS) != 0;
    const bool tiled = (prm->flags & CRT_FLAG_TILED_OUTPUT) != 0;
    const bool want_var = (prm->flags & CRT_FLAG_VARIANCE) != 0;
    if (prm->world > 1 && !tiled) return fail(CRT_ERR_INVALID_ARG, "crt_render: world > 1 needs CRT_FLAG_TILED_OUTPUT");
    if ((uint64_t)sc->dev.n_lights * (uint64_t)prm->light_sample_n > 0xffffu) return fail(CRT_ERR_UNSUPPORTED, "crt_render: more than 65535 next-event samples per vertex");
    try {
        HIP_CHECK(hipSetDevice(sc->device));
        Shard sh = make_shard(prm->width, prm->height, prm->world);
        const uint64_t max_items = std::min<uint64_t>(kMaxChunkItems, 1ull << std::min(30u, env_u32("CRT_CHUNK_LOG2", 30)));
        uint32_t chunk = (uint32_t)std::min<uint64_t>(s_count, std::max<uint64_t>(1, max_items / sh.nslots));
        uint64_t cap = (uint64_t)chunk * sh.nslots;
        const uint32_t pipeline = choose_pipeline(sc);
        RingPlan ring;
        std::memset(&ring, 0, sizeof(ring));
        if (pipeline == 4 && !want_stats && !want_var) {
            uint32_t shards = ITEM_SHARDS;
            while (shards < 1024u && sh.nslots / (shards * 2u) >= 1024u) shards *= 2u;
            const uint32_t spsh = ((sh.nslots + shards - 1) / shards + 63u) & ~63u;
            const uint64_t pool_slots = (uint64_t)sc->n_cus * 16u * (uint64_t)POOL3_P;
            uint32_t rs = 32;
            while (rs < 65536u && (uint64_t)rs * sh.nslots < 4ull * pool_slots) rs <<= 1;
            const uint32_t forced = env_u32("CRT_COMMIT_RING_LOG2", 0);
            if (forced) rs = 1u << std::min(16u, forced);
            const uint64_t per_shard = (uint64_t)spsh * s_count;
            const bool fits32 = per_shard * shards < 0xffffffffull;
            if ((forced || (prm->flags & CRT_FLAG_BOUNDED_RADIANCE)) && rs < s_count && fits32) {
                ring.samples = rs; ring.spsh = spsh; ring.shards = shards;
                chunk = s_count;
                cap = (uint64_t)rs * spsh * shards;
            }
        }
        const uint32_t pool_log2 = std::min(26u, std::max(8u, env_u32("CRT_POOL_LOG2", 22)));
        const uint32_t pool_n = (uint32_t)std::min<uint64_t>((cap + 255) / 256 * 256, 1ull << pool_log2);
        const int batch_max = (int)std::min<uint32_t>(kMaxBatch, env_u32("CRT_ROUND_BATCH", 16));
        int batch = batch_max;

        if (ring.samples) sc->ring_L.ensure_uncached(cap);
        else sc->L.ensure(cap);
        sc->last_radiance_bytes = cap * sizeof(float4);
        sc->last_ring_samples = ring.samples;
        sc->accum.ensure_uncached((size_t)sh.nslots * 3);
        const bool var_frame = want_var && (s_begin == 0 || (sc->var.valid && sc->var.samples == s_begin && sc->var.spp == prm->spp && sc->var.width == prm->width &&
                                                             sc->var.height == prm->height && sc->var.rank == prm->rank && sc->var.world == prm->world));
        sc->var.valid = false;
        if (want_var) sc->accum_q.ensure_uncached((size_t)sh.nslots * 3);
        auto accumulate = [&](const AParams& A, uint32_t samples_done) {
            if (want_var) launch_accumulate_var(A, sc->accum_q.p, st);
            else launch_accumulate(A, st);
            HIP_CHECK(hipGetLastError());
            if (!var_frame) return;
            sc->var.valid = true;
            sc->var.samples = samples_done; sc->var.spp = prm->spp; sc->var.width = prm->width; sc->var.height = prm->height;
            sc->var.rank = prm->rank; sc->var.world = prm->world; sc->var.tiled = tiled ? 1u : 0u;
        };
        const bool timing = stats != nullptr;
        if (timing && sc->ev.size() < (size_t)(4 * kMaxBatch + 4)) {
            while (sc->ev.size() < (size_t)(4 * kMaxBatch + 4)) {
                hipEvent_t e;
                HIP_CHECK(hipEventCreate(&e));
                sc->ev.push_back(e);
            }
        }
        const size_t counters_bytes = (size_t)CNT_SHARDS * CNT_STRIDE * sizeof(unsigned long long);
        HIP_CHECK(hipMemsetAsync(sc->counters.p, 0, counters_bytes, st));
        auto counter_sum = [&](int c) {
            unsigned long long v = 0;
            for (int s = 0; s < CNT_SHARDS; s++) v += sc->h_counters[s * CNT_STRIDE + c];
            return v;
        };
        unsigned long long alive_seen = 0;

        if (pipeline == 4) {
            const bool reference = prm->traversal == CRT_TRAVERSAL_REFERENCE;
            const bool exact = prm->traversal == CRT_TRAVERSAL_EXACT;
            const int mode_id = (reference ? 2 : exact ? 4 : 0) + (want_stats ? 1 : 0);
            const int mode3 = reference ? 1 : exact ? 2 : 0;
            const bool dec = use_dec(sc, mode3);
            const bool r16 = use_ref16(sc, mode3, dec);
            const bool impl = use_impl(sc, dec, r16);
            const Mega3Kernel kern3 = mega3_kernel(mode3, want_stats, mode3 != 1 && (prm->flags & CRT_FLAG_TRACE_ALL) != 0, false, r16, ring.samples != 0, dec, impl);
            const uint32_t pool_p = mega3_pool_p(dec, ring.samples != 0);
            MParams M;
            std::memset(&M, 0, sizeof(M));
            int per_cu = 1;
            uint32_t blocks, lanes;
            {
                auto q3 = [&](int* n) {
                    hipError_t e = hipOccupancyMaxActiveBlocksPerMultiprocessor(n, kern3, 64, 0);
                    if (e != hipSuccess || *n < 1) *n = 1;
                };
                q3(&per_cu);
                per_cu = (int)std::min<uint32_t>((uint32_t)per_cu, env_u32("CRT_MEGA_BLOCKS_PER_CU", 64));
                const uint64_t most_items = ring.samples ? (uint64_t)s_count * sh.nslots : cap;
                blocks = std::min<uint32_t>((uint32_t)std::min<uint64_t>((most_items + pool_p - 1) / pool_p, 0x7fffffffull), (uint32_t)(sc->n_cus * per_cu));
                lanes = blocks * pool_p;
            }
            sc->p_vx.ensure(lanes); sc->p_la.ensure(lanes); sc->p_cc.ensure(lanes); sc->p_id.ensure(lanes);
            sc->p_rec_a.ensure((size_t)lanes * CRT_BOUNCE_STACK_SIZE);
            sc->p_rec_b.ensure((size_t)lanes * CRT_BOUNCE_STACK_SIZE);
            const int lds_cap = mega3_lds_levels(dec, r16);
            const int spill_levels = r16 ? std::max(1, sc->stack_cap) : std::max(1, sc->stack_cap - lds_cap);
            sc->spill[0].ensure((size_t)spill_levels * lanes);
            Pool pool;
            std::memset(&pool, 0, sizeof(pool));
            pool.vx = sc->p_vx.p; pool.la = sc->p_la.p; pool.cc = sc->p_cc.p; pool.vn = sc->p_vn.p; pool.id = sc->p_id.p;
            pool.rec_a = sc->p_rec_a.p; pool.rec_b = sc->p_rec_b.p; pool.n = lanes;
            LParams P;
            std::memset(&P, 0, sizeof(P));
            P.sc = sc->dev; P.pool = pool;
            std::memcpy(P.eye, cam->eye, sizeof(P.eye));
            std::memcpy(P.inv_view, cam->inv_view, sizeof(P.inv_view));
            camera_scale_ar(cam, prm, P.scale, P.ar);
            P.width = prm->width; P.height = prm->height;
            P.p_rr = prm->p_rr; P.lsn = prm->light_sample_n; P.seed = prm->seed;
            P.rank = prm->rank; P.world = prm->world; P.tiles_x = sh.tiles_x; P.n_tiles = sh.n_tiles;
            P.nslots = sh.nslots;
            P.inv_lsn_pow2 = inv_if_pow2(prm->light_sample_n); P.lsn_div = make_fastdiv((uint32_t)std::max(1, prm->light_sample_n)); P.nslots_div = make_fastdiv(sh.nslots); P.tiles_x_div = make_fastdiv(sh.tiles_x);
            P.L = sc->L.p; P.counters = sc->counters.p; P.item_next = sc->item_next.p; P.n_mats = sc->n_mats;
            M.sc = sc->dev; M.counters = sc->counters.p; M.spill = sc->spill[0].p; M.spill_stride = lanes; M.stack_cap = lds_cap;
            AParams A;
            std::memset(&A, 0, sizeof(A));
            A.width = prm->width; A.height = prm->height; A.spp = prm->spp;
            A.rank = prm->rank; A.world = prm->world; A.tiles_x = sh.tiles_x; A.n_tiles = sh.n_tiles;
            A.nslots = sh.nslots; A.tiled_output = tiled ? 1 : 0;
            A.L = sc->L.p; A.accum = sc->accum.p;
            A.out_rgb = (uint8_t*)d_rgb; A.out_mean = (float*)d_mean;
            hipEvent_t e0 = nullptr, e1 = nullptr, e2 = nullptr, e3 = nullptr;
            if (timing) { e0 = sc->ev[0]; e1 = sc->ev[1]; e2 = sc->ev[2]; e3 = sc->ev[3]; HIP_CHECK(hipEventRecord(e0, st)); }
            double kernel_ms = 0.0;
            uint32_t launches = 0;
            for (uint32_t s0 = s_begin; s0 < s_end; s0 += chunk) {
                uint32_t ns = std::min(chunk, s_end - s0);
                P.sample_begin = s0;
                P.n_items = (uint32_t)((uint64_t)ns * sh.nslots);
                P.items_per_shard = ((P.n_items + ITEM_SHARDS - 1) / ITEM_SHARDS + 63u) & ~63u;
                if (ring.samples) {
                    P.items_per_shard = ring.spsh * ns;
                    P.n_items = P.items_per_shard * ring.shards;
                    P.ring_mask = ring.samples - 1u; P.spsh = ring.spsh; P.spsh_div = make_fastdiv(ring.spsh); P.ring_shards = ring.shards;
                    P.ring_stride = ring.spsh * ring.shards; P.n_samples = ns; P.tail_first = P.items_per_shard; P.spp_f = (float)prm->spp;
                    sc->ring_done.ensure_uncached((size_t)ring.shards * ring.samples);
                    sc->ring_state.ensure_uncached((size_t)ring.shards * ITEM_STRIDE);
                    P.ring_done = sc->ring_done.p; P.ring_state = sc->ring_state.p; P.accum = sc->accum.p; P.L = sc->ring_L.p;
                    std::vector<unsigned int>& state = sc->ring_state_host;
                    state.assign((size_t)ring.shards * ITEM_STRIDE, 0u);
                    for (uint32_t slot = 0; slot < sh.nslots; slot++) {
                        const uint32_t tile = (slot >> 6) * prm->world + prm->rank, pix = slot & 63u;
                        if (tile >= sh.n_tiles) continue;
                        const uint32_t ty = tile / sh.tiles_x, tx = tile - ty * sh.tiles_x;
                        if (tx * CRT_TILE + (pix & 7u) < prm->width && ty * CRT_TILE + (pix >> 3) < prm->height) state[(size_t)(slot / ring.spsh) * ITEM_STRIDE + 1]++;
                    }
                    HIP_CHECK(hipMemcpyAsync(sc->ring_state.p, state.data(), state.size() * sizeof(unsigned int), hipMemcpyHostToDevice, st));
                    HIP_CHECK(hipMemsetAsync(sc->ring_done.p, 0, (size_t)ring.shards * ring.samples * sizeof(unsigned int), st));
                }
                P.item_list = nullptr;
                {
                    const char* eo = std::getenv("CRT_ITEM_ORDER");
                    const bool order = !(eo && eo[0] == '0');
                    if (order && P.n_items > 0) {
                        P.order_window = std::min<uint32_t>(P.items_per_shard, env_u32("CRT_ORDER_WINDOW", 1u << 19));
                        if (ring.samples) {
                            P.order_window = std::min<uint32_t>(P.order_window, (ring.samples / 2u) * ring.spsh);
                            P.tail_first = P.items_per_shard - P.order_window;
                        }
                        P.items_per_shard_div = make_fastdiv(std::max(1u, P.items_per_shard));
                        const uint32_t n_sh = ring.samples ? ring.shards : (uint32_t)ITEM_SHARDS;
                        sc->item_list.ensure((size_t)n_sh * P.order_window);
                        sc->order_cnt.ensure((size_t)n_sh * 2 * 32);
                        HIP_CHECK(hipMemsetAsync(sc->order_cnt.p, 0, (size_t)n_sh * 2 * 32 * sizeof(unsigned int), st));
                        const uint32_t spans = (P.order_window + 1023u) / 1024u;
                        launch_order_items(ring.samples != 0, n_sh * spans, st, P, sc->item_list.p, sc->order_cnt.p);
                        HIP_CHECK(hipGetLastError());
                        P.item_list = sc->item_list.p;
                    }
                }
                P.items_per_shard_div = make_fastdiv(std::max(1u, P.items_per_shard));
                M.P = P;
                HIP_CHECK(hipMemsetAsync(sc->item_next.p, 0, (size_t)(ring.samples ? ring.shards : (uint32_t)ITEM_SHARDS) * ITEM_STRIDE * sizeof(unsigned int), st));
                if (timing) HIP_CHECK(hipEventRecord(e1, st));
                if (s0 == s_begin) HIP_CHECK(hipEventRecord(sc->ev_k0, st));
                {
                    MParams3 M3;
                    M3.M = M;
                    M3.spill = (int*)sc->spill[0].p;
                    M3.force_exact = (prm->flags & CRT_FLAG_FORCE_EXACT) ? 1u : 0u;
                    M3.dbg_loads = 0; M3.dbg_valu = 0;
                    if (!bbprof_launch(kern3, M3, blocks, st)) hipLaunchKernelGGL(kern3, dim3(blocks), dim3(64), 0, st, M3);
                }
                HIP_CHECK(hipGetLastError());
                if (s0 + ns >= s_end) HIP_CHECK(hipEventRecord(sc->ev_k1, st));
                if (timing) {
                    HIP_CHECK(hipEventRecord(e2, st));
                    HIP_CHECK(hipStreamSynchronize(st));
                    float ms = 0.0f;
                    HIP_CHECK(hipEventElapsedTime(&ms, e1, e2));
                    kernel_ms += ms;
                }
// ... 631 lines not shown
                        const uint32_t id = (uint32_t)newid[(size_t)t.ref[k]];
                        if (mixed[(size_t)t.ref[k]]) { if (n_m++ == 0) fm = id; } else { if (n_f++ == 0) ff = id; }
                    } else if (t.used[k]) {
                        const size_t dense = (size_t)(~t.ref[k]);
                        const size_t sparse = ni * 4 + (size_t)o;
                        for (int q = 0; q < 5; q++) lgi[sparse * 5 + (size_t)q] = leaf_geo[dense * 5 + (size_t)q];
                        rec_map[dense] = (int32_t)sparse;
                    }
                }
                if (mixed[i]) {
                    const uint32_t chunk[3] = {fm & 0xfffu, ((fm >> 12) & 7u) | ((ff & 0x1ffu) << 3), ((ff >> 9) & 63u) | (n_m << 6) | (n_f << 9)};
                    for (int a = 0; a < 3; a++) {
                        lo[0][a] = with_bits(lo[0][a], chunk[a], false);
                        hi[0][a] = with_bits(hi[0][a], chunk[a], true);
                        const float m = std::max(std::fabs(lo[0][a]), std::fabs(hi[0][a]));
                        cmax_i = std::max(cmax_i, m);
                    }
                }
                float4* o6 = &n4i[ni * (size_t)NODE4I_F4];
                for (int a = 0; a < 3; a++) {
                    o6[2 * a + 0] = make_float4(lo[0][a], lo[1][a], lo[2][a], lo[3][a]);
                    o6[2 * a + 1] = make_float4(hi[0][a], hi[1][a], hi[2][a], hi[3][a]);
                }
            }
            if (ok && cmax_i <= FLT_MAX) {
                const float pinf_ = std::numeric_limits<float>::infinity();
                for (int a = 0; a < 3; a++) { n4i[n4 * (size_t)NODE4I_F4 + 2 * (size_t)a] = make_float4(pinf_, pinf_, pinf_, pinf_); n4i[n4 * (size_t)NODE4I_F4 + 2 * (size_t)a + 1] = make_float4(-pinf_, -pinf_, -pinf_, -pinf_); }
                sc->nodes4i.upload(n4i); sc->leaf_geo_i.upload(lgi); sc->rec_map.upload(rec_map);
                sc->dev.nodes4i = sc->nodes4i.p; sc->dev.leaf_geo_i = sc->leaf_geo_i.p; sc->dev.rec_map = sc->rec_map.p;
                sc->dev.n_mixed4i = n_mixed;
                sc->dev.root4i = newid[0];
                sc->dev.empty4i_off = (uint32_t)(n4 * NODE4I_F4 * 16);
                coord_max = cmax_i;
                sc->impl_ok = true;
            }
        }
        sc->nodes4.upload(nodes4);
        sc->dev.nodes4 = sc->nodes4.p;
        sc->dev.root4 = root4;
        sc->dev.coord_max = coord_max;
        sc->depth4 = depth4;
        sc->accel.n_nodes4 = (uint32_t)n_nodes4; sc->accel.depth2 = (uint32_t)depth; sc->accel.depth4 = (uint32_t)depth4;
        sc->ref16_ok = n_nodes4 <= 32768 && leaf_geo.size() / 5 <= 32768;
        sc->ref16_inner_ok = n_nodes4 <= 32768;
        sc->dec_ok = leaf_geo.size() / 5 <= (size_t)LEAF_REC_MAX + 1;
        sc->accel.layout_caps = (sc->ref16_ok ? 1u : 0u) | (sc->ref16_inner_ok ? 2u : 0u) | (sc->dec_ok ? 4u : 0u) | (sc->impl_ok ? 8u : 0u);
        std::vector<float4> tri_nm(d->n_tris);
        for (uint32_t i = 0; i < d->n_tris; i++) {
            const crt_material& m = d->materials[d->tris[i].material];
            const int32_t w = (int32_t)((uint32_t)d->tris[i].material | (m.has_emit ? 1u << 30 : 0u) | (m.mode == 1 ? 1u << 31 : 0u));
            tri_nm[i] = make_float4(d->tris[i].normal[0], d->tris[i].normal[1], d->tris[i].normal[2], as_float(w));
        }
        sc->nodes3.upload(nodes3); sc->leaf_geo.upload(leaf_geo); sc->tri_nm.upload(tri_nm);
        sc->dev.tri_nm = sc->tri_nm.p;
        sc->max_leaf = max_leaf;
        sc->dev.nodes3 = sc->nodes3.p; sc->dev.leaf_geo = sc->leaf_geo.p;
        sc->dev.root3_fast = ref3(root_fast); sc->dev.root3_exact = ref3(root_exact);
        std::vector<uint4> lights(d->n_lights);
        for (uint32_t i = 0; i < d->n_lights; i++) {
            FastDiv fd = make_fastdiv(d->lights[i].count);
            lights[i] = make_uint4(d->lights[i].first_tri, d->lights[i].count, fd.m, fd.sh);
        }
        sc->nodes.upload(nodes); sc->tri_geo.upload(geo); sc->tri_mat.upload(tri_mat); sc->mats.upload(mats);
        sc->ltri.upload(ltri); sc->lights.upload(lights); sc->leaf_count.upload(leaf_count);
        sc->counters.alloc((size_t)CNT_SHARDS * CNT_STRIDE);
        sc->item_next.alloc((size_t)1024 * ITEM_STRIDE);
        sc->slot_next[0].alloc((size_t)SLOT_SHARDS * SLOT_STRIDE);
        sc->slot_next[1].alloc((size_t)SLOT_SHARDS * SLOT_STRIDE);
        HIP_CHECK(hipStreamCreateWithFlags(&sc->aux_stream, hipStreamNonBlocking));
        HIP_CHECK(hipEventCreateWithFlags(&sc->ev_fork, hipEventDisableTiming));
        HIP_CHECK(hipEventCreateWithFlags(&sc->ev_join, hipEventDisableTiming));
        HIP_CHECK(hipEventCreate(&sc->ev_k0));
        HIP_CHECK(hipEventCreate(&sc->ev_k1));
        {
            hipDeviceProp_t prop;
            HIP_CHECK(hipGetDeviceProperties(&prop, device));
            sc->n_cus = prop.multiProcessorCount > 0 ? prop.multiProcessorCount : 256;
        }
        HIP_CHECK(hipHostMalloc((void**)&sc->h_counters, (size_t)CNT_SHARDS * CNT_STRIDE * sizeof(unsigned long long), hipHostMallocDefault));
        sc->dev.nodes = sc->nodes.p; sc->dev.tri_geo = sc->tri_geo.p; sc->dev.tri_mat = sc->tri_mat.p; sc->dev.mats = sc->mats.p;
        sc->dev.ltri = sc->ltri.p; sc->dev.lights = sc->lights.p; sc->dev.leaf_count = sc->leaf_count.p;
        sc->dev.root_fast = root_fast; sc->dev.root_exact = root_exact; sc->dev.n_lights = (int32_t)d->n_lights;
        sc->n_tris = d->n_tris;
        sc->n_mats = d->n_materials;
        sc->stack_cap = std::max(depth + 2, 3 * sc->depth4 + 2);
        *out = sc;
        return CRT_OK;
    } catch (const HipFail& f) {
        delete sc;
        return fail_hip(f);
    } catch (const std::bad_alloc&) {
        delete sc;
        return fail(CRT_ERR_OOM, "crt_scene_create: out of host memory");
    }
}

int crt_scene_accel_info(crt_scene* sc, crt_accel_info* out)
{
    if (!sc || !out) return fail(CRT_ERR_INVALID_ARG, "crt_scene_accel_info: null argument");
    *out = sc->accel;
    return CRT_OK;
}

int crt_scene_export(crt_scene* sc, const char* name, void* dst, size_t capacity, size_t* bytes)
{
    if (!bytes) return fail(CRT_ERR_INVALID_ARG, "crt_scene_export: null bytes");
    static const char* names[] = {"nodes", "nodes3", "nodes4", "nodes4i", "leaf_geo", "leaf_geo_i", "rec_map", "tri_geo", "leaf_count", "tri_nm", "scalars"};
    int id = -1;
    for (int i = 0; name && i < 11; i++)
        if (std::strcmp(name, names[i]) == 0) id = i;
    if (id < 0) return fail(CRT_ERR_INVALID_ARG, std::string("crt_scene_export: unknown array ") + (name ? name : "(null)"));
    if (!sc) return fail(CRT_ERR_INVALID_ARG, "crt_scene_export: null scene");
    if (id == 10) {
        crt_tree_scalars s;
        std::memset(&s, 0, sizeof(s));
        s.root_fast = sc->dev.root_fast; s.root_exact = sc->dev.root_exact; s.root3_fast = sc->dev.root3_fast; s.root3_exact = sc->dev.root3_exact;
        s.root4 = sc->dev.root4; s.root4i = sc->impl_ok ? sc->dev.root4i : 0;
        s.n_mixed4i = sc->impl_ok ? sc->dev.n_mixed4i : 0; s.empty4_off = sc->dev.empty4_off; s.empty4i_off = sc->impl_ok ? sc->dev.empty4i_off : 0;
        s.coord_max = sc->dev.coord_max; s.stack_cap = (uint32_t)sc->stack_cap; s.node4i_f4 = NODE4I_F4;
        *bytes = sizeof(s);
        if (!dst) return CRT_OK;
        if (capacity < sizeof(s)) return fail(CRT_ERR_INVALID_ARG, "crt_scene_export: capacity below the size");
        std::memcpy(dst, &s, sizeof(s));
        return CRT_OK;
    }
    const bool leaf_root = sc->dev.root_fast < 0, impl = sc->impl_ok;
    const void* src = nullptr;
    size_t n = 0;
    switch (id) {
    case 0: src = sc->nodes.p; n = leaf_root ? 0 : sc->nodes.n * sizeof(float4); break;
    case 1: src = sc->nodes3.p; n = leaf_root ? 0 : sc->nodes3.n * sizeof(float4); break;
    case 2: src = sc->nodes4.p; n = sc->nodes4.n * sizeof(float4); break;
    case 3: src = sc->nodes4i.p; n = impl ? sc->nodes4i.n * sizeof(float4) : 0; break;
    case 4: src = sc->leaf_geo.p; n = sc->leaf_geo.n * sizeof(float4); break;
    case 5: src = sc->leaf_geo_i.p; n = impl ? sc->leaf_geo_i.n * sizeof(float4) : 0; break;
    case 6: src = sc->rec_map.p; n = impl ? sc->rec_map.n * sizeof(int32_t) : 0; break;
    case 7: src = sc->tri_geo.p; n = sc->tri_geo.n * sizeof(float4); break;
    case 8: src = sc->leaf_count.p; n = sc->leaf_count.n * sizeof(int32_t); break;
    default: src = sc->tri_nm.p; n = sc->tri_nm.n * sizeof(float4); break;
    }
    *bytes = n;
    if (!dst || n == 0) return CRT_OK;
    if (capacity < n) return fail(CRT_ERR_INVALID_ARG, "crt_scene_export: capacity below the size");
    try {
        HIP_CHECK(hipSetDevice(sc->device));
        HIP_CHECK(hipMemcpy(dst, src, n, hipMemcpyDeviceToHost));
        return CRT_OK;
    } catch (const HipFail& f) {
        return fail_hip(f);
    }
}

int crt_scene_destroy(crt_scene* sc)
{
    if (!sc) return CRT_OK;
    (void)hipSetDevice(sc->device);
    delete sc;
    return CRT_OK;
}

int crt_render_device(crt_scene* sc, const crt_camera* cam, const crt_params* prm, void* d_rgb, void* d_mean, void* stream, crt_stats* stats)
{
    return render_impl(sc, cam, prm, d_rgb, d_mean, (hipStream_t)stream, stats);
}

int crt_render(crt_scene* sc, const crt_camera* cam, const crt_params* prm, uint8_t* out_rgb, float* out_mean, crt_stats* stats)
{
    if (!sc || !prm || !out_rgb) return fail(CRT_ERR_INVALID_ARG, "crt_render: null argument");
    if (prm->world == 0 || prm->rank >= prm->world || prm->width == 0 || prm->height == 0) return fail(CRT_ERR_INVALID_ARG, "crt_render: bad shard or size");
    try {
        HIP_CHECK(hipSetDevice(sc->device));
        const bool tiled = (prm->flags & CRT_FLAG_TILED_OUTPUT) != 0;
        uint64_t npix = tiled ? make_shard(prm->width, prm->height, prm->world).nslots : (uint64_t)prm->width * prm->height;
        DevBuf<uint8_t> d_rgb;
        DevBuf<float> d_mean;
        d_rgb.alloc(npix * 3);
        if (out_mean) d_mean.alloc(npix * 3);
        int rc = render_impl(sc, cam, prm, d_rgb.p, out_mean ? d_mean.p : nullptr, nullptr, stats);
        if (rc != CRT_OK) return rc;
        HIP_CHECK(hipDeviceSynchronize());
        HIP_CHECK(hipMemcpy(out_rgb, d_rgb.p, npix * 3, hipMemcpyDeviceToHost));
        if (out_mean) HIP_CHECK(hipMemcpy(out_mean, d_mean.p, npix * 3 * sizeof(float), hipMemcpyDeviceToHost));
        return CRT_OK;
    } catch (const HipFail& f) {
        return fail_hip(f);
    }
}

int crt_render_range_device(crt_scene* sc, const crt_camera* cam, const crt_params* prm, uint32_t sample_begin, uint32_t sample_count,
                            void* d_rgb, void* d_mean, void* stream, crt_stats* stats)
{
    if (sample_count == 0xffffffffu) return fail(CRT_ERR_INVALID_ARG, "crt_render_range: bad sample count");
    return render_impl(sc, cam, prm, d_rgb, d_mean, (hipStream_t)stream, stats, sample_begin, sample_count);
}

int crt_render_range(crt_scene* sc, const crt_camera* cam, const crt_params* prm, uint32_t sample_begin, uint32_t sample_count,
                     uint8_t* out_rgb, float* out_mean, crt_stats* stats)
{
    if (!sc || !prm) return fail(CRT_ERR_INVALID_ARG, "crt_render_range: null argument");
    if (prm->world == 0 || prm->rank >= prm->world || prm->width == 0 || prm->height == 0) return fail(CRT_ERR_INVALID_ARG, "crt_render_range: bad shard or size");
    if (sample_count == 0xffffffffu || sample_count == 0 || (uint64_t)sample_begin + sample_count > prm->spp)
        return fail(CRT_ERR_INVALID_ARG, "crt_render_range: sample range outside [0, spp)");
    const bool last = sample_begin + sample_count == prm->spp;
    if (last && !out_rgb) return fail(CRT_ERR_INVALID_ARG, "crt_render_range: the range that ends at spp needs a frame buffer");
    try {
        HIP_CHECK(hipSetDevice(sc->device));
        const bool tiled = (prm->flags & CRT_FLAG_TILED_OUTPUT) != 0;
        uint64_t npix = tiled ? make_shard(prm->width, prm->height, prm->world).nslots : (uint64_t)prm->width * prm->height;
        DevBuf<uint8_t> d_rgb;
        DevBuf<float> d_mean;
        if (last) d_rgb.alloc(npix * 3);
        if (last && out_mean) d_mean.alloc(npix * 3);
        int rc = render_impl(sc, cam, prm, last ? d_rgb.p : nullptr, last && out_mean ? d_mean.p : nullptr, nullptr, stats, sample_begin, sample_count);
        if (rc != CRT_OK) return rc;
        HIP_CHECK(hipDeviceSynchronize());
        if (last) {
            HIP_CHECK(hipMemcpy(out_rgb, d_rgb.p, npix * 3, hipMemcpyDeviceToHost));
            if (out_mean) HIP_CHECK(hipMemcpy(out_mean, d_mean.p, npix * 3 * sizeof(float), hipMemcpyDeviceToHost));
        }
        return CRT_OK;
    } catch (const HipFail& f) {
        return fail_hip(f);
    }
}

int crt_last_launch_ms(crt_scene* sc, float* ms, uint32_t* launches)
{
    if (!sc || !ms) return fail(CRT_ERR_INVALID_ARG, "crt_last_launch_ms: null argument");
    if (sc->last_launches == 0) return fail(CRT_ERR_INVALID_ARG, "crt_last_launch_ms: no frame has been rendered by the megakernel on this handle");
    hipError_t e = hipEventElapsedTime(ms, sc->ev_k0, sc->ev_k1);
    if (e != hipSuccess) return fail(CRT_ERR_HIP, std::string("crt_last_launch_ms: hipEventElapsedTime: ") + hipGetErrorString(e) + " (synchronize the stream first)");
    if (launches) *launches = sc->last_launches;
    return CRT_OK;
}

int crt_radiance_storage(crt_scene* sc, uint64_t* bytes, uint32_t* ring_samples)
{
    if (!sc || !bytes) return fail(CRT_ERR_INVALID_ARG, "crt_radiance_storage: null argument");
    *bytes = sc->last_radiance_bytes;
    if (ring_samples) *ring_samples = sc->last_ring_samples;
    return CRT_OK;
}

static int variance_check(const crt_scene* sc, const void* out)
{
    if (!sc || !out) return fail(CRT_ERR_INVALID_ARG, "crt_variance: null argument");
    if (!sc->var.valid) return fail(CRT_ERR_INVALID_ARG, "crt_variance: no render with CRT_FLAG_VARIANCE on the handle yet, or the last render (or a range of the frame in flight) was submitted without it");
    if (sc->var.samples < 2) return fail(CRT_ERR_INVALID_ARG, "crt_variance: fewer than 2 samples accumulated (one sample has no variance)");
    return CRT_OK;
}

int crt_variance_device(crt_scene* sc, void* d_var, void* stream, uint32_t* samples_done)
{
    const int rc = variance_check(sc, d_var);
    if (rc != CRT_OK) return rc;
    try {
        HIP_CHECK(hipSetDevice(sc->device));
        Shard sh = make_shard(sc->var.width, sc->var.height, sc->var.world);
        AParams A;
        std::memset(&A, 0, sizeof(A));
        A.width = sc->var.width; A.height = sc->var.height; A.spp = sc->var.spp;
        A.rank = sc->var.rank; A.world = sc->var.world; A.tiles_x = sh.tiles_x; A.n_tiles = sh.n_tiles;
        A.nslots = sh.nslots; A.tiled_output = sc->var.tiled;
        A.accum = sc->accum.p;
        A.out_mean = (float*)d_var;
        launch_variance(A, sc->accum_q.p, (float)sc->var.samples, (float)sc->var.spp, (hipStream_t)stream);
        HIP_CHECK(hipGetLastError());
        if (samples_done) *samples_done = sc->var.samples;
        return CRT_OK;
    } catch (const HipFail& f) {
        return fail_hip(f);
    }
}

int crt_variance(crt_scene* sc, float* out_var, uint32_t* samples_done)
{
    const int rc0 = variance_check(sc, out_var);
    if (rc0 != CRT_OK) return rc0;
    try {
        HIP_CHECK(hipSetDevice(sc->device));
        const uint64_t npix = sc->var.tiled ? make_shard(sc->var.width, sc->var.height, sc->var.world).nslots : (uint64_t)sc->var.width * sc->var.height;
        DevBuf<float> d_var;
        d_var.alloc(npix * 3);
        const int rc = crt_variance_device(sc, d_var.p, nullptr, samples_done);
        if (rc != CRT_OK) return rc;
        HIP_CHECK(hipDeviceSynchronize());
        HIP_CHECK(hipMemcpy(out_var, d_var.p, npix * 3 * sizeof(float), hipMemcpyDeviceToHost));
        return CRT_OK;
    } catch (const HipFail& f) {
        return fail_hip(f);
    }
}

int crt_preview_device(crt_scene* sc, void* d_rgb, void* d_mean, void* stream, uint32_t* samples_done)
{
    if (!sc || !d_rgb) return fail(CRT_ERR_INVALID_ARG, "crt_preview: null argument");
    if (sc->acc.samples == 0) return fail(CRT_ERR_INVALID_ARG, "crt_preview: no progressive render in flight (submit a range that ends before spp first)");
    try {
        HIP_CHECK(hipSetDevice(sc->device));
        Shard sh = make_shard(sc->acc.width, sc->acc.height, sc->acc.world);
        AParams A;
        std::memset(&A, 0, sizeof(A));
        A.width = sc->acc.width; A.height = sc->acc.height; A.spp = sc->acc.spp;
        A.rank = sc->acc.rank; A.world = sc->acc.world; A.tiles_x = sh.tiles_x; A.n_tiles = sh.n_tiles;
        A.nslots = sh.nslots; A.tiled_output = sc->acc.tiled;
        A.accum = sc->accum.p;
        A.out_rgb = (uint8_t*)d_rgb; A.out_mean = (float*)d_mean;
        const float scale = (float)sc->acc.spp / (float)sc->acc.samples;
        launch_preview(A, scale, (hipStream_t)stream);
        HIP_CHECK(hipGetLastError());
        if (samples_done) *samples_done = sc->acc.samples;
        return CRT_OK;
    } catch (const HipFail& f) {
        return fail_hip(f);
    }
// ... 178 lines not shown
```

### include/crt.h

```cpp
#ifndef CRT_H
#define CRT_H

#include <stddef.h>
#include <stdint.h>

#ifdef __cplusplus
extern "C" {
#endif

#define CRT_ABI_VERSION 5

typedef enum {
    CRT_OK = 0,
    CRT_ERR_INVALID_ARG = -1,
    CRT_ERR_NO_DEVICE = -2,
    CRT_ERR_HIP = -3,
    CRT_ERR_UNSUPPORTED = -4,
    CRT_ERR_IO = -5,
    CRT_ERR_PARSE = -6,
    CRT_ERR_OOM = -7
} crt_status;

const char* crt_strerror(int status);
const char* crt_last_error(void);
// ... 30 lines not shown
} crt_light;

typedef struct {
    const crt_bvh_node* nodes;     uint32_t n_nodes;  int32_t root;
    const crt_triangle* tris;      uint32_t n_tris;
    const crt_material* materials; uint32_t n_materials;
    const crt_triangle* light_tris; uint32_t n_light_tris;
    const crt_light* lights;       uint32_t n_lights;
} crt_scene_desc;

typedef struct {
    float eye[3];
    float inv_view[9];
    float fov_y;
} crt_camera;

enum {
    CRT_TRAVERSAL_EXACT = 0,
    CRT_TRAVERSAL_REFERENCE = 1,
    CRT_TRAVERSAL_FAST = 2
};
enum {
    CRT_FLAG_STATS = 1u,
    CRT_FLAG_TILED_OUTPUT = 2u,
    CRT_FLAG_TRACE_ALL = 8u,
    CRT_FLAG_FORCE_EXACT = 4u,
    CRT_FLAG_BOUNDED_RADIANCE = 16u,
    CRT_FLAG_VARIANCE = 32u
};

typedef struct {
    uint32_t width, height;
    uint32_t spp;
    float p_rr;
    int32_t light_sample_n;
    uint64_t seed;
    uint32_t rank, world;
    uint32_t traversal;
    uint32_t flags;
} crt_params;

typedef struct {
    uint64_t paths;
    uint64_t rays;
    uint64_t shadow_rays, probe_rays;
    uint64_t inner_pops, leaf_pops, tri_tests, hits;
    uint64_t stack_sum, stack_max;
    uint64_t phase_cycles[24];
    float kernel_ms;
    float logic_ms;
    float total_ms;
    uint32_t kernel_launches;
    uint64_t rays_untraced;
} crt_stats;

typedef struct crt_scene crt_scene;

int crt_device_count(int* count);

int crt_scene_create(const crt_scene_desc* desc, int device, crt_scene** out);
typedef struct {
    uint32_t n_leaves, n_nodes2, n_nodes4, depth2, depth4;
    uint32_t sah_on_device;
    uint32_t index_splits;
    float sah_ms;
    float sah_device_ms;
    float runtime_init_ms;
    uint32_t layout_caps;
} crt_accel_info;
int crt_scene_accel_info(crt_scene* scene, crt_accel_info* out);
int crt_scene_destroy(crt_scene* scene);

int crt_shard_slots(uint32_t width, uint32_t height, uint32_t rank, uint32_t world, uint64_t* slots);

int crt_render(crt_scene* scene, const crt_camera* cam, const crt_params* params, uint8_t* out_rgb,
               float* out_mean, crt_stats* stats);

int crt_render_device(crt_scene* scene, const crt_camera* cam, const crt_params* params, void* d_rgb,
                      void* d_mean, void* hip_stream, crt_stats* stats);

int crt_last_launch_ms(crt_scene* scene, float* ms, uint32_t* launches);

int crt_radiance_storage(crt_scene* scene, uint64_t* bytes, uint32_t* ring_samples);

int crt_render_range(crt_scene* scene, const crt_camera* cam, const crt_params* params, uint32_t sample_begin,
                     uint32_t sample_count, uint8_t* out_rgb, float* out_mean, crt_stats* stats);
int crt_render_range_device(crt_scene* scene, const crt_camera* cam, const crt_params* params, uint32_t sample_begin,
                            uint32_t sample_count, void* d_rgb, void* d_mean, void* hip_stream, crt_stats* stats);

int crt_preview(crt_scene* scene, uint8_t* out_rgb, float* out_mean, uint32_t* samples_done);
int crt_preview_device(crt_scene* scene, void* d_rgb, void* d_mean, void* hip_stream, uint32_t* samples_done);

int crt_variance(crt_scene* scene, float* out_var, uint32_t* samples_done);
int crt_variance_device(crt_scene* scene, void* d_var, void* hip_stream, uint32_t* samples_done);

typedef struct { float* albedo; float* normal; float* depth; float* coverage; int32_t* tri; int32_t* material; } crt_aov_buffers;
typedef struct {
    uint64_t rays;
    uint32_t chunks;
    float total_ms;
} crt_aov_info;
int crt_render_aov(crt_scene* scene, const crt_camera* cam, const crt_params* params, const crt_aov_buffers* host_out, crt_aov_info* info);
int crt_render_aov_device(crt_scene* scene, const crt_camera* cam, const crt_params* params, const crt_aov_buffers* dev_out,
                          void* hip_stream, crt_aov_info* info);

typedef struct {
    uint32_t width, height;
    uint32_t iterations;
    float sigma_color, sigma_normal, sigma_albedo, sigma_depth;
} crt_denoise_params;
typedef struct { const float* color; const float* albedo; const float* normal; const float* depth; } crt_denoise_inputs;
typedef struct {
    float total_ms;
    uint32_t passes;
} crt_denoise_info;
int crt_denoise_defaults(crt_denoise_params* params);
int crt_denoise_scratch_bytes(uint32_t width, uint32_t height, uint64_t* bytes);
int crt_denoise(int device, const crt_denoise_params* params, const crt_denoise_inputs* host_in, float* out_mean, uint8_t* out_rgb,
                crt_denoise_info* info);
int crt_denoise_device(int device, const crt_denoise_params* params, const crt_denoise_inputs* dev_in, void* d_out_mean, void* d_out_rgb,
                       void* d_scratch, uint64_t scratch_bytes, void* hip_stream, crt_denoise_info* info);

typedef struct { const float* color; const float* variance; const float* albedo; const float* normal; const float* depth; } crt_denoise_var_inputs;
int crt_denoise_var_defaults(crt_denoise_params* params);
int crt_denoise_var(int device, const crt_denoise_params* params, const crt_denoise_var_inputs* host_in, float* out_mean, uint8_t* out_rgb,
                    float* out_variance, crt_denoise_info* info);
int crt_denoise_var_device(int device, const crt_denoise_params* params, const crt_denoise_var_inputs* dev_in, void* d_out_mean,
                           void* d_out_rgb, void* d_out_variance, void* d_scratch, uint64_t scratch_bytes, void* hip_stream,
                           crt_denoise_info* info);

typedef struct crt_multi crt_multi;
enum {
    CRT_GATHER_AUTO = 0,
    CRT_GATHER_RCCL = 1,
    CRT_GATHER_COPY = 2
};
typedef struct {
    uint32_t n_ranks;
    uint32_t gather;
    uint32_t rccl_ranks;
    int32_t rccl_version;
    float render_ms;
    float gather_ms;
    float frame_ms;
    float max_kernel_ms;
    uint64_t bytes_per_rank;
    uint64_t rays, paths, rays_untraced;
    char fallback_reason[160];
} crt_multi_info;
int crt_multi_create(const crt_scene_desc* desc, const int* devices, uint32_t n_devices, uint32_t gather, crt_multi** out);
int crt_multi_destroy(crt_multi* multi);
int crt_multi_render(crt_multi* multi, const crt_camera* cam, const crt_params* params, uint8_t* out_rgb, float* out_mean,
                     crt_stats* stats, crt_multi_info* info);
int crt_multi_frame_device(crt_multi* multi, void** d_rgb, void** d_mean, int* device);

#define CRT_INTERSECT_RAW_DIRECTIONS 0x100u
#define CRT_INTERSECT_FORCE_EXACT 0x200u
#define CRT_INTERSECT_VISIBILITY 0x400u
int crt_intersect(crt_scene* scene, uint32_t n, const float* origins, const float* dirs, uint32_t traversal,
                  int32_t* out_tri, float* out_t);

int crt_device_math(int device, const char* fn, uint32_t n, const float* a, const float* b, float* out);
int crt_device_philox(int device, uint32_t n, const uint32_t* ctr4, const uint32_t* key2, uint32_t* out4);
int crt_device_rcp_check(int device, uint64_t* mismatches, uint64_t* outside);
typedef struct {
    int32_t root_fast, root_exact, root3_fast, root3_exact, root4, root4i;
// ... 53 lines not shown
```

Baseline: 13210.

## Pack path state into one word of the cc record to cut per-lane loads

Adds a packed path-state form that puts depth, stage, a flag, the NEE sample index and the triangle id into the w word of the per-lane cc float4, so logic stages can often skip loading the la record. The cosine term moves out of rec_b.w into its own cosn array. The aim is fewer global memory loads and stores per path step in the megakernel. In exchange the code gains bit-width checks and branches, and keeps a fallback path when the scene's triangle or light counts do not fit.

```diff
diff --git a/cudaraytracing_amd/_capi.py b/cudaraytracing_amd/_capi.py
--- a/cudaraytracing_amd/_capi.py
+++ b/cudaraytracing_amd/_capi.py
@@ -166,7 +166,7 @@
 ABI_VERSION = 5
 
 EXPORTS = ["crt_strerror", "crt_last_error", "crt_abi_version", "crt_device_count", "crt_scene_create",
-           "crt_scene_accel_info", "crt_scene_destroy", "crt_task_obj", "crt_shard_slots", "crt_render", "crt_render_device", "crt_render_range", "crt_render_range_device", "crt_last_launch_ms", "crt_radiance_storage", "crt_preview", "crt_preview_device", "crt_variance", "crt_variance_device", "crt_render_aov", "crt_render_aov_device", "crt_denoise_defaults", "crt_denoise_scratch_bytes", "crt_denoise", "crt_denoise_device", "crt_denoise_var_defaults", "crt_denoise_var", "crt_denoise_var_device", "crt_multi_create", "crt_multi_destroy",
+           "crt_scene_accel_info", "crt_scene_destroy", "crt_task_obj", "crt_shard_slots", "crt_render", "crt_render_device", "crt_render_range", "crt_render_range_device", "crt_last_launch_ms", "crt_radiance_storage", "crt_state_pack_widths", "crt_path_state_form", "crt_preview", "crt_preview_device", "crt_variance", "crt_variance_device", "crt_render_aov", "crt_render_aov_device", "crt_denoise_defaults", "crt_denoise_scratch_bytes", "crt_denoise", "crt_denoise_device", "crt_denoise_var_defaults", "crt_denoise_var", "crt_denoise_var_device", "crt_multi_create", "crt_multi_destroy",
            "crt_multi_render", "crt_multi_frame_device", "crt_intersect",
            "crt_device_math", "crt_device_philox", "crt_device_rcp_check", "crt_scene_export", "crt_host_scene_create", "crt_host_scene_destroy",
            "crt_host_scene_add_obj", "crt_host_scene_set_bvh", "crt_host_scene_set_bvh_device", "crt_host_scene_desc", "crt_host_scene_num_objects",
@@ -205,6 +205,8 @@
                                           C.c_void_p, C.c_void_p, C.POINTER(Stats)]
     L.crt_last_launch_ms.argtypes = [C.c_void_p, C.POINTER(C.c_float), C.POINTER(C.c_uint32)]
     L.crt_radiance_storage.argtypes = [C.c_void_p, C.POINTER(C.c_uint64), C.POINTER(C.c_uint32)]
+    L.crt_state_pack_widths.argtypes = [C.c_uint64, C.c_uint64, C.POINTER(C.c_uint32), C.POINTER(C.c_uint32)]
+    L.crt_path_state_form.argtypes = [C.c_void_p, C.POINTER(C.c_uint32), C.POINTER(C.c_uint32), C.POINTER(C.c_uint32)]
     L.crt_preview.argtypes = [C.c_void_p, C.c_void_p, C.c_void_p, C.POINTER(C.c_uint32)]
     L.crt_preview_device.argtypes = [C.c_void_p, C.c_void_p, C.c_void_p, C.c_void_p, C.POINTER(C.c_uint32)]
     L.crt_variance.argtypes = [C.c_void_p, C.c_void_p, C.POINTER(C.c_uint32)]
diff --git a/cudaraytracing_amd/api.py b/cudaraytracing_amd/api.py
--- a/cudaraytracing_amd/api.py
+++ b/cudaraytracing_amd/api.py
@@ -258,6 +258,11 @@
         ms, n = C.c_float(), C.c_uint32()
         capi.check(capi.lib().crt_last_launch_ms(self._handle("last_launch_ms"), C.byref(ms), C.byref(n)), "crt_last_launch_ms")
         return float(ms.value), int(n.value)
+
+    def path_state_form(self):
+        p, q, t = C.c_uint32(0), C.c_uint32(0), C.c_uint32(0)
+        capi.check(capi.lib().crt_path_state_form(self._handle("path_state_form"), C.byref(p), C.byref(q), C.byref(t)), "crt_path_state_form")
+        return bool(p.value), int(q.value), int(t.value)
 
     def radiance_storage(self):
         b, r = C.c_uint64(), C.c_uint32()
diff --git a/cudaraytracing_amd/csrc/crt_mega3.h b/cudaraytracing_amd/csrc/crt_mega3.h
--- a/cudaraytracing_amd/csrc/crt_mega3.h
+++ b/cudaraytracing_amd/csrc/crt_mega3.h
@@ -103,7 +103,7 @@
     int32_t dbg_loads, dbg_valu;
 };
 
-static_assert(offsetof(MParams3, dbg_loads) == 748 && offsetof(MParams3, dbg_valu) == 752, "tools/bbprof/instrument.py reads the counter buffer's address from these two kernel-argument dwords");
+static_assert(offsetof(MParams3, dbg_loads) == 756 && offsetof(MParams3, dbg_valu) == 760, "tools/bbprof/instrument.py reads the counter buffer's address from these two kernel-argument dwords");
 
 
 typedef void (*Mega3Kernel)(const MParams3);
diff --git a/cudaraytracing_amd/csrc/crt_mega3.hip b/cudaraytracing_amd/csrc/crt_mega3.hip
--- a/cudaraytracing_amd/csrc/crt_mega3.hip
+++ b/cudaraytracing_amd/csrc/crt_mega3.hip
@@ -145,7 +145,7 @@
         for (int j = 0; j < CRT_FINISH_PF; j++) {
             const int vj = v - j > 0 ? v - j : 0;
             a[j] = gld_rec(&pl.rec_a[(size_t)vj * pl.n + slot]);
-            cs[j] = __uint_as_float(gld((const uint32_t*)&pl.rec_b[(size_t)vj * pl.n + slot].w));
+            cs[j] = __uint_as_float(gld((const uint32_t*)&pl.cosn[(size_t)vj * pl.n + slot]));
         }
 #pragma unroll
         for (int j = 0; j < CRT_FINISH_PF; j++) fm[j] = mat_row(tb, TNM_MAT(__float_as_uint(a[j].w)), 0);
@@ -166,6 +166,25 @@
 __device__ __forceinline__ bool shadow_blocked_bit(const bool tl_inf, const int tri) { return tri >= 0 || tl_inf; }
 #define ST_TL_INF (1u << 12)
 
+#ifdef CRT_ASM_ST_PACK
+#define ST_PACK_OF(P_) ((uint32_t)(CRT_ASM_ST_PACK))
+#else
+#define ST_PACK_OF(P_) ((P_).st_pack)
+#endif
+struct PState { uint32_t depth, stage, q, tri; bool flag; };
+__device__ __forceinline__ PState unpack_state(const uint32_t pk, const uint32_t w)
+{
+    const uint32_t tb = pk & 31u, qb = (pk >> 8) & 31u;
+    PState s;
+    s.depth = w >> STP_DEPTH_SHIFT; s.stage = (w >> STP_STAGE_SHIFT) & 7u; s.flag = (w & STP_FLAG) != 0u;
+    s.tri = w & ((1u << tb) - 1u); s.q = (w >> tb) & ((1u << qb) - 1u);
+    return s;
+}
+__device__ __forceinline__ float pack_state(const uint32_t pk, const uint32_t depth, const uint32_t stage, const bool flag, const uint32_t q, const uint32_t tri)
+{
+    return __uint_as_float((depth << STP_DEPTH_SHIFT) | (stage << STP_STAGE_SHIFT) | (flag ? STP_FLAG : 0u) | (q << (pk & 31u)) | tri);
+}
+
 template <int MODE, bool RING = false>
 __device__ __forceinline__ uint32_t logic_A(const LParams& P, const Tables<false>& tb, const uint32_t g, const float4 qa, const float4 qb, NewRay& nr,
                                             PathCounters& cnt, const bool trace_all)
@@ -173,12 +192,18 @@
     const DevScene& sc = P.sc;
     const Pool& pl = P.pool;
     constexpr bool TRI_CC = MODE != 1;
-    const float4 la = gld(&pl.la[g]);
+    const uint32_t pk = TRI_CC ? ST_PACK_OF(P) : 0u;
+    const uint32_t n_nee = (uint32_t)(sc.n_lights * P.lsn);
+    const float4 cc = gld(&pl.cc[g]);
     const uint4 idv = load_path_id<RING, !TRI_CC>(P, g);
-    const float4 cc = gld(&pl.cc[g]);
+    float4 la = make_float4(0.0f, 0.0f, 0.0f, 0.0f);
+    if (!pk || n_nee > 2u) la = gld(&pl.la[g]);
+    const PState ps = unpack_state(pk, __float_as_uint(cc.w));
     const uint32_t st = __float_as_uint(la.w);
-    const uint32_t stage = (st >> 8) & 15u;
-    const uint32_t vtri_old = TRI_CC ? ((st & 0xfffu) == ((uint32_t)ST_HIT << 8) ? 0u : __float_as_uint(cc.w)) : idv.w;
+    const uint32_t stage = pk ? ps.stage : (st >> 8) & 15u;
+    const uint32_t depth_in = pk ? ps.depth : st & 255u, q_in = pk ? ps.q : st >> 16;
+    const bool tl_inf = pk ? ps.flag : (st & ST_TL_INF) != 0u;
+    const uint32_t vtri_old = pk ? ps.tri : TRI_CC ? ((st & 0xfffu) == ((uint32_t)ST_HIT << 8) ? 0u : __float_as_uint(cc.w)) : idv.w;
     const float4 vn = gld(&sc.tri_nm[vtri_old]);
     const float res_t = qa.w;
     const int res_tri = __float_as_int(qb.w);
@@ -187,8 +212,7 @@
     const uint32_t mat_cur = stage == ST_HIT ? TNM_MAT(__float_as_uint(gq_hit.w)) : mat_old;
     uint32_t tnm_cur = stage == ST_HIT ? __float_as_uint(gq_hit.w) : __float_as_uint(vn.w);
     float4 m0_cur = mat_row(tb, mat_cur, 0);
-    const uint32_t n_nee = (uint32_t)(sc.n_lights * P.lsn);
-    const uint32_t q_next = stage == ST_SHADOW ? (st >> 16) + 1 : 0u;
+    const uint32_t q_next = stage == ST_SHADOW ? q_in + 1 : 0u;
     uint4 lg_next = make_uint4(0u, 1u, 0u, 0u);
     if (n_nee > 0) {
         if (sc.n_lights == 1) {
@@ -197,8 +221,9 @@
         } else lg_next = gld(&tb.lights[fast_div(q_next < n_nee ? q_next : 0u, P.lsn_div.m, P.lsn_div.sh)]);
     }
     Lane s;
-    s.depth = st & 255u; s.q = st >> 16; s.stage = stage;
+    s.depth = depth_in; s.q = q_in; s.stage = stage;
     s.Ld = f3(la.x, la.y, la.z);
+    if (pk && q_in == 0u) s.Ld = f3(0.0f, 0.0f, 0.0f);
     s.nrm = f3(vn.x, vn.y, vn.z); s.mat = TNM_MAT(__float_as_uint(vn.w));
     s.pixel_index = idv.x; s.k = idv.y; s.item = idv.z;
     s.ro = f3(qa.x, qa.y, qa.z); s.tl = 0.0f;
@@ -206,7 +231,7 @@
     s.pos = s.ro; s.vtri = vtri_old; s.c = f3(0.0f, 0.0f, 0.0f); s.kind = RAY_NONE;
     bool do_enter = false;
     if (stage == ST_SHADOW) {
-        const bool blocked = TRI_CC ? shadow_blocked_bit((st & ST_TL_INF) != 0u, res_tri) : shadow_blocked<MODE>(cc.w, res_t, res_tri);
+        const bool blocked = TRI_CC ? shadow_blocked_bit(tl_inf, res_tri) : shadow_blocked<MODE>(cc.w, res_t, res_tri);
         if (!blocked) s.Ld = add3(s.Ld, f3(cc.x, cc.y, cc.z));
         s.q++;
     } else if (stage == ST_HIT) {
@@ -217,7 +242,7 @@
             const F3 pn = s.nrm;
             float cos_prev = dot3(unit3(sub3(pos, s.ro)), pn);
             cos_prev = cos_prev > 0.0f ? cos_prev : 0.0f;
-            gst_rec(&pl.rec_b[pr].w, cos_prev);
+            gst_rec(&pl.cosn[pr], cos_prev);
             if (TNM_SPECULAR(__float_as_uint(vn.w))) {
                 const float ns = mat_row(tb, s.mat, 0).w;
                 const float4 pb = gld_rec(&pl.rec_b[pr]);
@@ -230,7 +255,8 @@
                 const F3 refd = unit3(sample_lobe(out, d_theta, d_phi, rng_uniform(rp.x), rng_uniform(rp.y)));
                 gst_rec(&pl.rec_b[(size_t)s.depth * pl.n + g], make_float4(s.rd.x, s.rd.y, s.rd.z, 0.0f));
                 gst(&pl.vx[g], make_float4(pos.x, pos.y, pos.z, __int_as_float(res_tri)));
-                gst(&pl.la[g], make_float4(s.Ld.x, s.Ld.y, s.Ld.z, __uint_as_float(s.depth | ((uint32_t)ST_PROBE << 8) | (s.q << 16))));
+                if (pk) gst(&pl.cc[g], make_float4(0.0f, 0.0f, 0.0f, pack_state(pk, s.depth, ST_PROBE, false, 0u, vtri_old)));
+                else gst(&pl.la[g], make_float4(s.Ld.x, s.Ld.y, s.Ld.z, __uint_as_float(s.depth | ((uint32_t)ST_PROBE << 8) | (s.q << 16))));
                 nr.o = s.ro; nr.d = unit3(refd);  nr.tl = 0.0f; nr.kind = RAY_CLOSEST; nr.flags = RF_PROBE;
                 return PH3_NONE;
             }
@@ -275,14 +301,18 @@
         if (TNM_SPECULAR(tnm_cur)) gst_rec(&pl.rec_b[(size_t)s.depth * pl.n + g], make_float4(s.rd.x, s.rd.y, s.rd.z, 0.0f));
         if (!TRI_CC) store_path_tri(P, g, s.vtri);
         if (TNM_EMITTER(tnm_cur)) {
-            gst(&pl.la[g], make_float4(TRI_CC ? __uint_as_float(s.vtri) : 0.0f, 0.0f, 0.0f, __uint_as_float(s.depth | ((uint32_t)ST_FIN << 8) | (1u << 16))));
+            if (pk) gst(&pl.cc[g], make_float4(0.0f, 0.0f, 0.0f, pack_state(pk, s.depth, ST_FIN, true, 0u, s.vtri)));
+            else gst(&pl.la[g], make_float4(TRI_CC ? __uint_as_float(s.vtri) : 0.0f, 0.0f, 0.0f, __uint_as_float(s.depth | ((uint32_t)ST_FIN << 8) | (1u << 16))));
             return PH3_LC;
         }
         s.Ld = f3(0.0f, 0.0f, 0.0f);
         s.q = 0;
         if (n_nee == 0) {
-            gst(&pl.la[g], make_float4(0.0f, 0.0f, 0.0f, __uint_as_float(s.depth | ((uint32_t)ST_NEED << 8))));
-            if (TRI_CC) gst(&pl.cc[g].w, __uint_as_float(s.vtri));
+            if (pk) gst(&pl.cc[g], make_float4(0.0f, 0.0f, 0.0f, pack_state(pk, s.depth, ST_NEED, false, 0u, s.vtri)));
+            else {
+                gst(&pl.la[g], make_float4(0.0f, 0.0f, 0.0f, __uint_as_float(s.depth | ((uint32_t)ST_NEED << 8))));
+                if (TRI_CC) gst(&pl.cc[g].w, __uint_as_float(s.vtri));
+            }
             nr.o = s.pos;
             return PH3_LB;
         }
@@ -300,14 +330,22 @@
         cnt.rays++; cnt.shadow++;
         s.q++;
         if (s.q == n_nee) {
-            gst(&pl.la[g], make_float4(s.Ld.x, s.Ld.y, s.Ld.z, __uint_as_float(s.depth | ((uint32_t)ST_NEED << 8))));
-            if (TRI_CC) gst(&pl.cc[g].w, __uint_as_float(s.vtri));
+            if (pk) gst(&pl.cc[g], make_float4(s.Ld.x, s.Ld.y, s.Ld.z, pack_state(pk, s.depth, ST_NEED, false, 0u, s.vtri)));
+            else {
+                gst(&pl.la[g], make_float4(s.Ld.x, s.Ld.y, s.Ld.z, __uint_as_float(s.depth | ((uint32_t)ST_NEED << 8))));
+                if (TRI_CC) gst(&pl.cc[g].w, __uint_as_float(s.vtri));
+            }
             nr.o = s.pos;
             return PH3_LB;
         }
     }
-    gst(&pl.la[g], make_float4(s.Ld.x, s.Ld.y, s.Ld.z, __uint_as_float(s.depth | ((uint32_t)ST_SHADOW << 8) | (s.q << 16) | ((TRI_CC && s.tl == pinf()) ? ST_TL_INF : 0u))));
-    gst(&pl.cc[g], make_float4(s.c.x, s.c.y, s.c.z, TRI_CC ? __uint_as_float(s.vtri) : s.tl));
+    if (pk) {
+        gst(&pl.cc[g], make_float4(s.c.x, s.c.y, s.c.z, pack_state(pk, s.depth, ST_SHADOW, s.tl == pinf(), s.q, s.vtri)));
+        if (s.q >= 1u) gst(&pl.la[g], make_float4(s.Ld.x, s.Ld.y, s.Ld.z, 0.0f));
+    } else {
+        gst(&pl.la[g], make_float4(s.Ld.x, s.Ld.y, s.Ld.z, __uint_as_float(s.depth | ((uint32_t)ST_SHADOW << 8) | (s.q << 16) | ((TRI_CC && s.tl == pinf()) ? ST_TL_INF : 0u))));
+        gst(&pl.cc[g], make_float4(s.c.x, s.c.y, s.c.z, TRI_CC ? __uint_as_float(s.vtri) : s.tl));
+    }
     nr.o = s.ro; nr.d = s.rd; nr.tl = s.tl; nr.kind = RAY_SHADOW;
     nr.flags = RF_SHADOW | (s.q + 1 == n_nee ? RF_LAST : 0u) | (skip ? RF_SKIP : 0u);
     return PH3_NONE;
@@ -318,17 +356,21 @@
 {
     const Pool& pl = P.pool;
     constexpr bool TRI_CC = MODE != 1;
+    const uint32_t pk = TRI_CC ? ST_PACK_OF(P) : 0u;
     const float4 la = gld(&pl.la[g]);
     const uint4 idv = load_path_id<RING, !TRI_CC>(P, g);
     const float4 cc = gld(&pl.cc[g]);
+    const PState ps = unpack_state(pk, __float_as_uint(cc.w));
     const uint32_t st = __float_as_uint(la.w);
-    const uint32_t stage = (st >> 8) & 15u;
-    uint32_t depth = st & 255u;
+    const uint32_t stage = pk ? ps.stage : (st >> 8) & 15u;
+    uint32_t depth = pk ? ps.depth : st & 255u;
+    const uint32_t vtri = pk ? ps.tri : TRI_CC ? __float_as_uint(cc.w) : idv.w;
     F3 Ld = f3(la.x, la.y, la.z);
+    if (pk && ps.q == 0u) Ld = f3(0.0f, 0.0f, 0.0f);
     if (stage == ST_SHADOW) {
-        const bool blocked = TRI_CC ? shadow_blocked_bit((st & ST_TL_INF) != 0u, __float_as_int(qb.w)) : shadow_blocked<MODE>(cc.w, qa.w, __float_as_int(qb.w));
+        const bool blocked = TRI_CC ? shadow_blocked_bit(pk ? ps.flag : (st & ST_TL_INF) != 0u, __float_as_int(qb.w)) : shadow_blocked<MODE>(cc.w, qa.w, __float_as_int(qb.w));
         if (!blocked) Ld = add3(Ld, f3(cc.x, cc.y, cc.z));
-    }
+    } else if (pk) Ld = f3(cc.x, cc.y, cc.z);
     bool stop = depth == CRT_BOUNCE_STACK_SIZE - 1;
     U4 rb;
     rb.x = rb.y = rb.z = rb.w = 0;
@@ -337,15 +379,17 @@
         stop = rng_uniform(rb.x) > P.p_rr;
     }
     if (stop) {
-        gst(&pl.la[g], make_float4(Ld.x, Ld.y, Ld.z, __uint_as_float(depth | ((uint32_t)ST_FIN << 8))));
+        if (pk) gst(&pl.cc[g], make_float4(Ld.x, Ld.y, Ld.z, pack_state(pk, depth, ST_FIN, false, 0u, vtri)));
+        else gst(&pl.la[g], make_float4(Ld.x, Ld.y, Ld.z, __uint_as_float(depth | ((uint32_t)ST_FIN << 8))));
         return PH3_LC;
     }
-    const float4 vn = gld(&P.sc.tri_nm[TRI_CC ? __float_as_uint(cc.w) : idv.w]);
+    const float4 vn = gld(&P.sc.tri_nm[vtri]);
     const float4 vx = qa;
     gst_rec(&pl.rec_a[(size_t)depth * pl.n + g], make_float4(Ld.x, Ld.y, Ld.z, vn.w));
     const F3 ndir = unit3(sample_hemisphere(f3(vn.x, vn.y, vn.z), rng_uniform(rb.y), rng_uniform(rb.z)));
     depth++;
-    gst(&pl.la[g], make_float4(Ld.x, Ld.y, Ld.z, __uint_as_float(depth | ((uint32_t)ST_HIT << 8))));
+    if (pk) gst(&pl.cc[g], make_float4(Ld.x, Ld.y, Ld.z, pack_state(pk, depth, ST_HIT, false, 0u, vtri)));
+    else gst(&pl.la[g], make_float4(Ld.x, Ld.y, Ld.z, __uint_as_float(depth | ((uint32_t)ST_HIT << 8))));
     nr.o = f3(vx.x, vx.y, vx.z); nr.d = unit3(ndir);  nr.tl = 0.0f; nr.kind = RAY_CLOSEST; nr.flags = 0;
     return PH3_NONE;
 }
@@ -356,11 +400,14 @@
 {
     constexpr bool TRI_CC = MODE != 1;
     const Pool& pl = P.pool;
-    const float4 la = gld(&pl.la[g]);
+    const uint32_t pk = TRI_CC ? ST_PACK_OF(P) : 0u;
+    float4* const sp = pk ? pl.cc : pl.la;
+    const float4 la = gld(&sp[g]);
     const uint4 idv = load_path_id<RING, !TRI_CC>(P, g);
+    const PState ps = unpack_state(pk, __float_as_uint(la.w));
     const uint32_t st = __float_as_uint(la.w);
-    const uint32_t stage = (st >> 8) & 15u;
-    const uint32_t depth = st & 255u;
+    const uint32_t stage = pk ? ps.stage : (st >> 8) & 15u;
+    const uint32_t depth = pk ? ps.depth : st & 255u;
     constexpr bool ring = RING;
     const bool waiting = ring && stage == ST_WAIT;
     const uint32_t home_ = RING ? blockIdx.x & (P.ring_shards - 1u) : blockIdx.x & (ITEM_SHARDS - 1);
@@ -378,12 +425,12 @@
         bool emissive = false;
         F3 ke = f3(0.0f, 0.0f, 0.0f);
         if (stage == ST_HIT) deepest = (int)depth - 1;
-        else if ((st >> 16) & 1u) {
+        else if (pk ? ps.flag : ((st >> 16) & 1u) != 0u) {
             emissive = true;
-            const float4 m2 = mat_row(tb, TNM_MAT(__float_as_uint(gld(&P.sc.tri_nm[TRI_CC ? __float_as_uint(la.x) : idv.w]).w)), 2);
+            const float4 m2 = mat_row(tb, TNM_MAT(__float_as_uint(gld(&P.sc.tri_nm[pk ? ps.tri : TRI_CC ? __float_as_uint(la.x) : idv.w]).w)), 2);
             ke = f3(m2.x, m2.y, m2.z);
         }
-        const F3 L = finish_path_m3(P, tb, g, deepest, emissive, ke, stage == ST_FIN && !emissive, f3(la.x, la.y, la.z));
+        const F3 L = finish_path_m3(P, tb, g, deepest, emissive, ke, (stage == ST_FIN && !emissive) || (TRI_CC && stage == ST_HIT), f3(la.x, la.y, la.z));
         if (ring) {
             const uint32_t sh = fast_div(idv.z, P.items_per_shard_div.m, P.items_per_shard_div.sh), c = idv.z - sh * P.items_per_shard;
             const uint32_t s = fast_div(c, P.spsh_div.m, P.spsh_div.sh), rs = s & P.ring_mask;
@@ -422,14 +469,14 @@
         if (ring && !ring_gate_open(P, item, home_, home_word_)) {
             if (!waiting) {
                 store_path_id<!TRI_CC>(P, g, item);
-                gst(&pl.la[g], make_float4(0.0f, 0.0f, 0.0f, __uint_as_float((uint32_t)ST_WAIT << 8)));
+                gst(&sp[g], make_float4(0.0f, 0.0f, 0.0f, pk ? pack_state(pk, 0u, ST_WAIT, false, 0u, 0u) : __uint_as_float((uint32_t)ST_WAIT << 8)));
             }
             return LC_WAIT;
         }
         cnt.paths++;
         if (!waiting) store_path_id<!TRI_CC>(P, g, item);
         const F3 wd = camera_dir(P, pixel_index, k, pi, pj);
-        gst(&pl.la[g], make_float4(0.0f, 0.0f, 0.0f, __uint_as_float((uint32_t)ST_HIT << 8)));
+        gst(&sp[g], make_float4(0.0f, 0.0f, 0.0f, pk ? pack_state(pk, 0u, ST_HIT, false, 0u, 0u) : __uint_as_float((uint32_t)ST_HIT << 8)));
         nr.o = f3(P.eye[0], P.eye[1], P.eye[2]); nr.d = unit3(wd);  nr.tl = 0.0f; nr.kind = RAY_CLOSEST; nr.flags = 0;
         return LC_RAY;
     }
@@ -912,7 +959,8 @@
         const int n_valid = __builtin_amdgcn_readfirstlane((int)min((uint32_t)LDS3::P, pl.n > base ? pl.n - base : 0u));
         for (int i = lane; i < n_valid; i += 64) {
             S.rq(PH3_LC)[i] = (uint8_t)i;
-            pl.la[base + i] = make_float4(0.0f, 0.0f, 0.0f, __uint_as_float((uint32_t)ST_NEW << 8));
+            if (MODE != 1 && !QUERY && ST_PACK_OF(P)) pl.cc[base + i] = make_float4(0.0f, 0.0f, 0.0f, pack_state(ST_PACK_OF(P), 0u, ST_NEW, false, 0u, 0u));
+            else pl.la[base + i] = make_float4(0.0f, 0.0f, 0.0f, __uint_as_float((uint32_t)ST_NEW << 8));
         }
         qn[PH3_LC] = n_valid;
     }
diff --git a/cudaraytracing_amd/csrc/crt_path.h b/cudaraytracing_amd/csrc/crt_path.h
--- a/cudaraytracing_amd/csrc/crt_path.h
+++ b/cudaraytracing_amd/csrc/crt_path.h
@@ -23,9 +23,25 @@
 #define ITEM_STRIDE 32
 
 enum { ST_DEAD = 0, ST_NEW = 1, ST_HIT = 2, ST_PROBE = 3, ST_SHADOW = 4, ST_FIN = 5, ST_NEED = 6, ST_WAIT = 7, ST_COUNT_ };
-static_assert(ST_COUNT_ <= 16, "a stage is kept in 4 bits");
+static_assert(ST_COUNT_ <= 16, "two-word path state: a stage is kept in 4 bits");
 enum { RAY_NONE = 0, RAY_CLOSEST = 1, RAY_SHADOW = 2 };
 #define ITEM_NONE 0xffffffffu
+
+#define STP_DEPTH_SHIFT 26
+#define STP_STAGE_SHIFT 23
+#define STP_FLAG (1u << 22)
+#define STP_FIELD_BITS 22
+static_assert(CRT_BOUNCE_STACK_SIZE <= 64 && ST_COUNT_ <= 8, "packed path state: 6 bits of depth, 3 bits of stage");
+#define ST_PACK_ON 0x80000000u
+inline uint32_t bits_of(uint32_t x) { uint32_t b = 0; while (x) { b++; x >>= 1; } return b; }
+inline bool state_pack_widths(uint64_t n_nee, uint64_t n_triangles, uint32_t* qbits, uint32_t* tbits)
+{
+    if (n_nee > 0xffffffffull || n_triangles > 0x100000000ull) return false;
+    const uint32_t qb = bits_of((uint32_t)n_nee), tb = bits_of(n_triangles ? (uint32_t)(n_triangles - 1) : 0u);
+    if (qb + tb > STP_FIELD_BITS) return false;
+    *qbits = qb; *tbits = tb;
+    return true;
+}
 
 struct Pool {
     float4* ro;
@@ -38,6 +54,7 @@
     float2* res;
     float4* rec_a;
     float4* rec_b;
+    float* cosn;
     uint32_t n;
 };
 
@@ -51,7 +68,7 @@
     float p_rr;
     int32_t lsn;
     float inv_lsn_pow2;
-    uint32_t pad_;
+    uint32_t st_pack;
     uint64_t seed;
     uint32_t rank, world, tiles_x, n_tiles;
     uint32_t nslots;
diff --git a/cudaraytracing_amd/csrc/crt_render.hip b/cudaraytracing_amd/csrc/crt_render.hip
--- a/cudaraytracing_amd/csrc/crt_render.hip
+++ b/cudaraytracing_amd/csrc/crt_render.hip
@@ -32,6 +32,7 @@
     DevBuf<uint4> p_id;
     uint32_t n_mats = 0;
     DevBuf<float2> p_res;
+    DevBuf<float> p_cosn;
     DevBuf<float> accum;
     DevBuf<float4> aov_acc;
     DevBuf<unsigned long long> counters;
@@ -41,6 +42,7 @@
     DevBuf<float4> ring_L;
     std::vector<unsigned int> ring_state_host;
     uint64_t last_radiance_bytes = 0;
+    uint32_t last_state_pack = 0;
     uint32_t last_ring_samples = 0;
     DevBuf<unsigned int> order_cnt;
     DevBuf<unsigned int> slot_next[2];
@@ -270,6 +272,21 @@
     if (!dec || !r16 || !sc->impl_ok) return false;
     const char* e = std::getenv("CRT_IMPL");
     return !(e && e[0] == '0');
+}
+struct StateForm { bool fits; uint32_t q_bits, tri_bits; };
+static StateForm state_form_of_call(crt_scene* sc, int32_t lsn)
+{
+    StateForm f{false, 0u, 0u};
+    f.fits = state_pack_widths((uint64_t)sc->dev.n_lights * (uint64_t)std::max(0, lsn), sc->n_tris, &f.q_bits, &f.tri_bits);
+    sc->accel.layout_caps = (sc->accel.layout_caps & ~16u) | (f.fits ? 0u : 16u);
+    return f;
+}
+static uint32_t choose_state_pack(const StateForm& f, int mode)
+{
+    if (mode == 1 || !f.fits) return 0u;
+    const char* e = std::getenv("CRT_STATE_PACK");
+    if (e && e[0] == '0') return 0u;
+    return ST_PACK_ON | (f.q_bits << 8) | f.tri_bits;
 }
 uint32_t choose_pipeline(const crt_scene* sc);
 
@@ -388,6 +405,8 @@
         uint32_t chunk = (uint32_t)std::min<uint64_t>(s_count, std::max<uint64_t>(1, max_items / sh.nslots));
         uint64_t cap = (uint64_t)chunk * sh.nslots;
         const uint32_t pipeline = choose_pipeline(sc);
+        const StateForm state_form = state_form_of_call(sc, prm->light_sample_n);
+        sc->last_state_pack = 0u;
         RingPlan ring;
         std::memset(&ring, 0, sizeof(ring));
         if (pipeline == 4 && !want_stats && !want_var) {
@@ -475,13 +494,14 @@
             sc->p_vx.ensure(lanes); sc->p_la.ensure(lanes); sc->p_cc.ensure(lanes); sc->p_id.ensure(lanes);
             sc->p_rec_a.ensure((size_t)lanes * CRT_BOUNCE_STACK_SIZE);
             sc->p_rec_b.ensure((size_t)lanes * CRT_BOUNCE_STACK_SIZE);
+            sc->p_cosn.ensure((size_t)lanes * CRT_BOUNCE_STACK_SIZE);
             const int lds_cap = mega3_lds_levels(dec, r16);
             const int spill_levels = r16 ? std::max(1, sc->stack_cap) : std::max(1, sc->stack_cap - lds_cap);
             sc->spill[0].ensure((size_t)spill_levels * lanes);
             Pool pool;
             std::memset(&pool, 0, sizeof(pool));
             pool.vx = sc->p_vx.p; pool.la = sc->p_la.p; pool.cc = sc->p_cc.p; pool.vn = sc->p_vn.p; pool.id = sc->p_id.p;
-            pool.rec_a = sc->p_rec_a.p; pool.rec_b = sc->p_rec_b.p; pool.n = lanes;
+            pool.rec_a = sc->p_rec_a.p; pool.rec_b = sc->p_rec_b.p; pool.cosn = sc->p_cosn.p; pool.n = lanes;
             LParams P;
             std::memset(&P, 0, sizeof(P));
             P.sc = sc->dev; P.pool = pool;
@@ -490,6 +510,8 @@
             camera_scale_ar(cam, prm, P.scale, P.ar);
             P.width = prm->width; P.height = prm->height;
             P.p_rr = prm->p_rr; P.lsn = prm->light_sample_n; P.seed = prm->seed;
+            P.st_pack = choose_state_pack(state_form, mode3);
+            sc->last_state_pack = P.st_pack;
             P.rank = prm->rank; P.world = prm->world; P.tiles_x = sh.tiles_x; P.n_tiles = sh.n_tiles;
             P.nslots = sh.nslots;
             P.inv_lsn_pow2 = inv_if_pow2(prm->light_sample_n); P.lsn_div = make_fastdiv((uint32_t)std::max(1, prm->light_sample_n)); P.nslots_div = make_fastdiv(sh.nslots); P.tiles_x_div = make_fastdiv(sh.tiles_x);
@@ -1287,6 +1309,7 @@
         sc->dev.ltri = sc->ltri.p; sc->dev.lights = sc->lights.p; sc->dev.leaf_count = sc->leaf_count.p;
         sc->dev.root_fast = root_fast; sc->dev.root_exact = root_exact; sc->dev.n_lights = (int32_t)d->n_lights;
         sc->n_tris = d->n_tris;
+        (void)state_form_of_call(sc, 1);
         sc->n_mats = d->n_materials;
         sc->stack_cap = std::max(depth + 2, 3 * sc->depth4 + 2);
         *out = sc;
@@ -1436,6 +1459,21 @@
     hipError_t e = hipEventElapsedTime(ms, sc->ev_k0, sc->ev_k1);
     if (e != hipSuccess) return fail(CRT_ERR_HIP, std::string("crt_last_launch_ms: hipEventElapsedTime: ") + hipGetErrorString(e) + " (synchronize the stream first)");
     if (launches) *launches = sc->last_launches;
+    return CRT_OK;
+}
+
+int crt_state_pack_widths(uint64_t n_nee, uint64_t n_triangles, uint32_t* q_bits, uint32_t* tri_bits)
+{
+    if (!q_bits || !tri_bits) return fail(CRT_ERR_INVALID_ARG, "crt_state_pack_widths: null argument");
+    return state_pack_widths(n_nee, n_triangles, q_bits, tri_bits) ? CRT_OK : CRT_ERR_UNSUPPORTED;
+}
+
+int crt_path_state_form(crt_scene* sc, uint32_t* packed, uint32_t* q_bits, uint32_t* tri_bits)
+{
+    if (!sc || !packed) return fail(CRT_ERR_INVALID_ARG, "crt_path_state_form: null argument");
+    *packed = sc->last_state_pack != 0u ? 1u : 0u;
+    if (q_bits) *q_bits = (sc->last_state_pack >> 8) & 31u;
+    if (tri_bits) *tri_bits = sc->last_state_pack & 31u;
     return CRT_OK;
 }
 
diff --git a/include/crt.h b/include/crt.h
--- a/include/crt.h
+++ b/include/crt.h
@@ -136,6 +136,9 @@
 int crt_last_launch_ms(crt_scene* scene, float* ms, uint32_t* launches);
 
 int crt_radiance_storage(crt_scene* scene, uint64_t* bytes, uint32_t* ring_samples);
+
+int crt_state_pack_widths(uint64_t n_nee, uint64_t n_triangles, uint32_t* q_bits, uint32_t* tri_bits);
+int crt_path_state_form(crt_scene* scene, uint32_t* packed, uint32_t* q_bits, uint32_t* tri_bits);
 
 int crt_render_range(crt_scene* scene, const crt_camera* cam, const crt_params* params, uint32_t sample_begin,
                      uint32_t sample_count, uint8_t* out_rgb, float* out_mean, crt_stats* stats);
```

After: 13490, median of 6. 1.02x the previous value.
